# teofum/yart

Measured on AMD Instinct MI355X. Metric: Msamples/sec (W*H*spp/s), Sponza-class 1080p 8-bounce, higher is better.
Workload: dtype f32; 1 GPU; sponza_class (generated atrium, 264356 triangles, env-lit) 1920x1080, 256 spp, 8 bounces; pipeline=wavefront, tiles=64x64 pixel blocks, Morton order, round-robin over ranks, pipeline_flags=2

## Files before the change

### yart_amd/csrc/stream_kernels.inc

```

struct SamplerTabArgs {
  SamplerConfig cfg;
  const uint32_t* pixels; uint32_t nPixels, dims;
  uint64_t* entries; uint64_t* hash; uint32_t* sobol1;
  const uint32_t* matrix52;
};
__global__ void __launch_bounds__(kBlock) k_sampler_tables(SamplerTabArgs a) {
  const uint32_t gtid = blockIdx.x * blockDim.x + threadIdx.x, stride = gridDim.x * blockDim.x;
  for (uint32_t k = gtid; k < a.dims + 3u; k += stride) a.hash[k] = hashDim(k);
  for (uint32_t k = gtid; k < 8u * 256u; k += stride) {
    const uint32_t b = k >> 8, v = k & 255u;
    uint32_t x = 0;
    for (uint32_t j = 0; j < 8; j++) if (((v >> j) & 1u) && 8u * b + j < 52u) x ^= a.matrix52[8u * b + j];
    a.sobol1[k] = x;
  }
  const uint64_t total = uint64_t(a.dims) * a.nPixels;
  for (uint64_t k = gtid; k < total; k += stride) {
    const uint32_t pi = uint32_t(k / a.dims), dim = uint32_t(k - uint64_t(pi) * a.dims);
    const uint32_t pk = a.pixels[pi];
    a.entries[k] = samplerTableEntry(a.cfg, encodeMorton2(pk & 0xffffu, pk >> 16), dim);
  }
}

__global__ void __launch_bounds__(kBlock) k_wf_generate(WfArgs a) {
  WF_DYN(a);
  const uint32_t* sobol = reinterpret_cast<const uint32_t*>(a.sc.lut + LutDev::sobol);
  __shared__ SamplerLds smpLds;
  samplerToLds(a.rc.sampler, smpLds, true);
  for (uint32_t i = blockIdx.x * blockDim.x + threadIdx.x; i < a.nPaths; i += gridDim.x * blockDim.x) {
    const uint32_t pi = i / a.spp, s = i - pi * a.spp;
    const uint32_t pk = a.pixels[pi];
    wfGenerate(a.rc, sobol, a.cam, pk & 0xffffu, pk >> 16, s + a.sampleOffset, a.pixBase + pi, a.st, i);
    a.qA[i] = i;
  }
}

__global__ void __launch_bounds__(kBlock) k_wf_refill(WfArgs a) {
  const uint32_t* sobol = reinterpret_cast<const uint32_t*>(a.sc.lut + LutDev::sobol);
  __shared__ SamplerLds smpLds;
  samplerToLds(a.rc.sampler, smpLds, true);
  const uint32_t lane = threadIdx.x & 63u;
  const uint32_t waveId = (blockIdx.x * blockDim.x + threadIdx.x) >> 6, nWaves = (gridDim.x * blockDim.x) >> 6;
  const uint32_t per = (((a.poolSlots + nWaves - 1u) / nWaves) + 63u) & ~63u;
  const uint32_t s0 = waveId * per < a.poolSlots ? waveId * per : a.poolSlots, s1 = s0 + per < a.poolSlots ? s0 + per : a.poolSlots;
  uint32_t nFree = 0;
  for (uint32_t base = s0; base < s1; base += 64u) {
    const uint32_t slot = base + lane;
    nFree += uint32_t(__popcll(__ballot(slot < s1 && a.slotMap[slot] == kWfFreeSlot)));
  }
  uint32_t first = 0, avail = 0;
  if (nFree != 0u && a.counters[WC_STARTED] < a.nPaths) {
    if (lane == 0) first = atomicAdd(&a.counters[WC_STARTED], nFree);
    first = __shfl(first, 0);
    avail = first < a.nPaths ? (a.nPaths - first < nFree ? a.nPaths - first : nFree) : 0u;
  }
  uint32_t taken = 0;
  for (uint32_t base = s0; base < s1; base += 64u) {
    const uint32_t slot = base + lane;
    const bool isFree = slot < s1 && a.slotMap[slot] == kWfFreeSlot;
    const unsigned long long m = __ballot(isFree);
    const uint32_t k = taken + uint32_t(__popcll(m & ((1ull << lane) - 1ull)));
    const bool take = isFree && k < avail;
    if (take) {
      const uint32_t i = first + k;
      const uint32_t pi = i / a.spp, sm = i - pi * a.spp;
      const uint32_t pk = a.pixels[pi];
      wfGenerate(a.rc, sobol, a.cam, pk & 0xffffu, pk >> 16, sm + a.sampleOffset, a.pixBase + pi, a.st, slot);
      a.slotMap[slot] = i;
    }
    if (slot < s1) a.qA[slot] = (isFree && !take) ? kWfFreeSlot : slot;
    taken += uint32_t(__popcll(m));
  }
  const uint32_t live = (s1 - s0) - nFree + avail;
  if (lane == 0 && live != 0u) atomicAdd(&a.counters[WC_NEXT], live);
}
__global__ void k_wf_pool_advance(uint32_t* counters, uint32_t poolSlots) {
  if (threadIdx.x == 0 && blockIdx.x == 0) {
    counters[WC_ACTIVE] = poolSlots;
    for (uint32_t k = 1; k < WC_COUNT; k++) if (k != WC_STARTED) counters[k] = 0;
  }
}
__global__ void k_wf_pool_init(uint32_t* slotMap, uint32_t n) {
  for (uint32_t i = blockIdx.x * blockDim.x + threadIdx.x; i < n; i += gridDim.x * blockDim.x) slotMap[i] = kWfFreeSlot;
}

__global__ void k_wf_reset_retry(uint32_t* counters) {
  if (threadIdx.x == 0 && blockIdx.x == 0) { counters[WC_RETRY] = 0; counters[WC_CUR_RETRY] = 0; counters[WC_RESUME] = 0; }
}

#ifndef YART_COMPACT_NUM
#define YART_COMPACT_NUM 1
#define YART_COMPACT_DEN 2
#endif
__device__ __forceinline__ bool wfCompactPlan(const WfArgs& a, const WfDyn& d, uint32_t count, uint32_t& dst) {
  dst = d.inTail == 1u ? 1u : 0u;
  return count > 0u && count <= a.tailCap[dst] && uint64_t(YART_COMPACT_DEN) * count <= uint64_t(YART_COMPACT_NUM) * d.extent;
}
__global__ void __launch_bounds__(kBlock) k_wf_compact(WfArgs a) {
  const WfDyn d = *a.dyn;
  const uint32_t count = a.counters[WC_ACTIVE];
  uint32_t dst;
  if (!wfCompactPlan(a, d, count, dst)) return;
  const WfState from = d.st, to = a.tail[dst];
  uint32_t* map = a.tailMap[dst];
  const uint32_t stride = gridDim.x * blockDim.x;
  for (uint32_t k0 = blockIdx.x * blockDim.x + threadIdx.x; k0 < count; k0 += 2u * stride) {
    const uint32_t k1 = k0 + stride;
    const bool v1 = k1 < count;
    const uint32_t s0 = a.qA[k0], s1 = v1 ? a.qA[k1] : s0;
    const f4 a0 = wfLd(from.ray0 + s0), b0 = wfLd(from.ray1 + s0), c0 = wfLd(from.thr + s0), d0 = wfLd(from.acc + s0), e0 = wfLd(from.hit1 + s0);
    const f4 a1 = wfLd(from.ray0 + s1), b1 = wfLd(from.ray1 + s1), c1 = wfLd(from.thr + s1), d1 = wfLd(from.acc + s1), e1 = wfLd(from.hit1 + s1);
    const uint32_t m0 = d.slotMap ? d.slotMap[s0] : s0, m1 = d.slotMap ? d.slotMap[s1] : s1;
    wfSt(to.ray0 + k0, a0); wfSt(to.ray1 + k0, b0); wfSt(to.thr + k0, c0); wfSt(to.acc + k0, d0); wfSt(to.hit1 + k0, e0);
    map[k0] = m0; a.qA[k0] = k0;
    if (v1) {
      wfSt(to.ray0 + k1, a1); wfSt(to.ray1 + k1, b1); wfSt(to.thr + k1, c1); wfSt(to.acc + k1, d1); wfSt(to.hit1 + k1, e1);
      map[k1] = m1; a.qA[k1] = k1;
    }
  }
}
__global__ void k_wf_compact_commit(WfArgs a) {
  if (threadIdx.x != 0 || blockIdx.x != 0) return;
  const WfDyn d = *a.dyn;
  const uint32_t count = a.counters[WC_ACTIVE];
  uint32_t dst;
  if (!wfCompactPlan(a, d, count, dst)) return;
  WfDyn n;
  n.st = a.tail[dst]; n.slotMap = a.tailMap[dst]; n.extent = count; n.inTail = dst + 1u;
  *a.dyn = n;
}

__global__ void k_wf_advance(uint32_t* counters, unsigned long long* pathsLog) {
  if (threadIdx.x == 0 && blockIdx.x == 0) {
    counters[0] = counters[1];
    if (pathsLog) *pathsLog += counters[1] - counters[WC_DUMMY];
    for (uint32_t k = 1; k < WC_COUNT; k++) if (k != WC_STARTED) counters[k] = 0;
  }
}

__global__ void __launch_bounds__(kBlock) k_wf_roulette(WfArgs a) {
  WF_EMPTY_BLOCK(a.counters[WC_SHADOW], kBlock);
  WF_DYN(a);
  const uint32_t count = a.counters[WC_SHADOW];
  const uint32_t stride = gridDim.x * blockDim.x;
  const uint32_t rounds = (count + stride - 1) / stride;
  __shared__ uint32_t stageNext[kBlock / 64][kStageCap];
  WaveStage sNext{stageNext[threadIdx.x >> 6], 0};
  __shared__ SamplerLds smpLds;
  samplerToLds(a.rc.sampler, smpLds, false);
  for (uint32_t r = 0; r < rounds; r++) {
    const uint32_t k = r * stride + blockIdx.x * blockDim.x + threadIdx.x;
    bool toNext = false;
    uint32_t slot = 0;
    if (k < count) {
      slot = a.qS[k];
      if (a.poolSlots) {
        const uint32_t fl = asU(wfLd1(&a.st.acc[slot].w));
        if ((fl & WF_DEPTH_MASK) >= 2u && !(fl & WF_FINAL)) toNext = wfRouletteAfterShadow(a.rc, a.st, slot, fl & WF_DEPTH_MASK, a.L, a.slotMap, true);
      } else toNext = wfRouletteAfterShadow(a.rc, a.st, slot, a.bounce + 1u, a.L, a.slotMap, false);
    }
    if (!a.poolSlots) sNext.push(a.qB, &a.counters[WC_NEXT], toNext, slot);
  }
  sNext.flush(a.qB, &a.counters[WC_NEXT]);
}
```

### yart_amd/csrc/wavefront.hpp

```cpp
#pragma once
#include "integrator.hpp"

namespace yart_hip {

struct WfState {
  f4 *ray0, *ray1, *thr, *acc, *hit0, *hit1, *sh0, *sh1, *sh2;
};
struct WfTally {
#if defined(YART_COUNT_TRAVERSAL)
  uint32_t box = 0, tri = 0, trav = 0, shade = 0;
  uint32_t resumed = 0;
  uint32_t waste = 0;
  uint32_t flipAlive = 0, flipDead = 0;
#endif
#if defined(YART_TRACE_STATS)
  uint32_t ph[16] = {0, 0, 0, 0, 0, 0, 0, 0, 0, 0, 0, 0, 0, 0, 0, 0};
#endif
};
#if defined(YART_TRACE_STATS)
#define WF_PHASE(t, k)                                                                  \
  do {                                                                                  \
    const unsigned long long _m = __ballot(true);                                       \
    (t).ph[2 * (k)] += (int(threadIdx.x & 63u) == __ffsll((long long) _m) - 1) ? 1u : 0u; \
    (t).ph[2 * (k) + 1] += 1u;                                                          \
  } while (0)
#else
#define WF_PHASE(t, k) ((void)0)
#endif
#if defined(YART_COUNT_TRAVERSAL)
#define WF_TALLY_TRAV(t, ac) ((t).box += (ac).nBox, (t).tri += (ac).nTri, (t).trav += (ac).nTrav)
#define WF_TALLY_SHADE(t) ((t).shade++)
#define WF_TALLY_FLIP(t, toAlive) ((toAlive) ? (t).flipAlive++ : (t).flipDead++)
#else
#define WF_TALLY_TRAV(t, ac) ((void)0)
#define WF_TALLY_SHADE(t) ((void)0)
#define WF_TALLY_FLIP(t, toAlive) ((void)0)
#endif

#if defined(YART_SHADE_REGIONS) && defined(__HIPCC__)
constexpr int kShadeRegions = 16;
static __device__ unsigned long long g_shadeRegion[3 * kShadeRegions];
#endif
#if defined(YART_SHADE_REGIONS) && defined(__HIP_DEVICE_COMPILE__)
__shared__ unsigned long long srAcc[16][3 * kShadeRegions];
__shared__ unsigned long long srLast[16];
#define SR_MARK(k)                                                                       \
  do {                                                                                   \
    const unsigned long long _m = __ballot(true);                                        \
    if (int(threadIdx.x & 63u) == __ffsll((long long) _m) - 1) {                         \
      const unsigned long long _t = clock64();                                           \
      unsigned long long* _a = srAcc[threadIdx.x >> 6];                                  \
      _a[k] += _t - srLast[threadIdx.x >> 6]; _a[kShadeRegions + (k)] += 1ull;           \
      _a[2 * kShadeRegions + (k)] += (unsigned long long) __popcll(_m);                  \
      srLast[threadIdx.x >> 6] = clock64();                                              \
    }                                                                                    \
  } while (0)
#else
#define SR_MARK(k) ((void)0)
#endif

enum : uint32_t { WF_SPECULAR = 1u << 8, WF_REGULARIZED = 1u << 9, WF_MISS = 1u << 10, WF_DEPTH_MASK = 0xffu,
                  WF_NEE_SHIFT = 16, WF_NEE_ONE = 1u << 16, WF_NEE_MASK = 0xffu << 16,
                  WF_FINAL = 1u << 11, WF_ATT_NAN = 1u << 12,
                  WF_RR_PENDING = 1u << 13, WF_DEAD = 1u << 14 };

constexpr uint32_t kWfNodeBits = 20, kWfClassBits = 11, kWfClassMiss = (1u << kWfClassBits) - 1u;
YART_HD uint32_t wfHitWord(const HitRec& h, bool didHit) {
  if (!didHit) return kWfClassMiss << kWfNodeBits;
  return h.node | ((h.backSide >> 1) << kWfNodeBits) | ((h.backSide & 1u) << 31);
}
YART_HD float asF(uint32_t u) { return __builtin_bit_cast(float, u); }
YART_HD uint32_t asU(float f) { return __builtin_bit_cast(uint32_t, f); }
YART_HD f4 mk4(float x, float y, float z, float w) { f4 r; r.x = x; r.y = y; r.z = z; r.w = w; return r; }

#if defined(__HIP_DEVICE_COMPILE__) && !defined(YART_NO_NT_STATE)
typedef float wf_v4 __attribute__((ext_vector_type(4)));
typedef __attribute__((address_space(1))) wf_v4 wf_v4_global;
typedef __attribute__((address_space(1))) float wf_f_global;
__device__ __forceinline__ f4 wfLd(const f4* p) {
  const wf_v4 v = __builtin_nontemporal_load((const wf_v4_global*) reinterpret_cast<const wf_v4*>(p));
  return mk4(v.x, v.y, v.z, v.w);
}
__device__ __forceinline__ void wfSt(f4* p, f4 v) {
  wf_v4 q; q.x = v.x; q.y = v.y; q.z = v.z; q.w = v.w;
  __builtin_nontemporal_store(q, (wf_v4_global*) reinterpret_cast<wf_v4*>(p));
}
__device__ __forceinline__ void wfSt1(float* p, float v) { __builtin_nontemporal_store(v, (wf_f_global*) p); }
__device__ __forceinline__ float wfLd1(const float* p) { return *(const wf_f_global*) p; }
#else
YART_HD f4 wfLd(const f4* p) { return *p; }
YART_HD void wfSt(f4* p, f4 v) { *p = v; }
YART_HD void wfSt1(float* p, float v) { *p = v; }
YART_HD float wfLd1(const float* p) { return *p; }
#endif

struct WfPath {
  f3 o, d, att, L;
  float lastPdf, accRoughness;
  uint32_t flags, slot;
  Sampler smp;
};
YART_HD WfPath wfLoad(const WfState& s, uint32_t i) {
  const f4 r0 = wfLd(s.ray0 + i), r1 = wfLd(s.ray1 + i), t = wfLd(s.thr + i), a = wfLd(s.acc + i), h1 = wfLd(s.hit1 + i);
  WfPath p;
  p.o = mk3(r0.x, r0.y, r0.z); p.d = mk3(r0.w, r1.x, r1.y); p.lastPdf = r1.z; p.accRoughness = r1.w;
  p.att = mk3(t.x, t.y, t.z); p.smp.dim = asU(t.w); p.L = mk3(a.x, a.y, a.z); p.flags = asU(a.w);
  p.smp.morton = uint64_t(asU(h1.y)) | (uint64_t(asU(h1.z)) << 32); p.smp.pix = asU(h1.w); p.slot = i;
  return p;
}
YART_HD void wfStoreRay(const WfState& s, uint32_t i, const WfPath& p) {
  wfSt(s.ray0 + i, mk4(p.o.x, p.o.y, p.o.z, p.d.x));
  wfSt(s.ray1 + i, mk4(p.d.y, p.d.z, p.lastPdf, p.accRoughness));
}
YART_HD void wfStoreThr(const WfState& s, uint32_t i, const WfPath& p) {
  wfSt(s.thr + i, mk4(p.att.x, p.att.y, p.att.z, asF(p.smp.dim)));
  wfSt(s.acc + i, mk4(p.L.x, p.L.y, p.L.z, asF(p.flags)));
}
YART_HD uint32_t wfPathRays(uint32_t flags) { return (flags & WF_DEPTH_MASK) + ((flags & WF_NEE_MASK) >> WF_NEE_SHIFT); }

YART_HD bool wfRoulette(const RenderConst& rc, WfPath& p) {
  const uint32_t depth = p.flags & WF_DEPTH_MASK;
  if (depth > 1 && maxComponent(p.att) < 1.0f) {
    float q = stdmax(0.0f, 1.0f - maxComponent(p.att));
    if (get1D(p.smp, rc.sampler) < q) return false;
    p.att /= 1.0f - q;
  }
  return depth < rc.maxDepth;
}
YART_HD bool wfRouletteTentative(const RenderConst& rc, WfPath& p) {
  if (!(maxComponent(p.att) < 1.0f)) return true;
  const float q = stdmax(0.0f, 1.0f - maxComponent(p.att));
  p.flags |= WF_RR_PENDING;
  if (get1D(p.smp, rc.sampler) < q) { p.flags |= WF_FINAL; return false; }
  return true;
}
YART_HD void wfRouletteScale(f3& att) {
  const float q = stdmax(0.0f, 1.0f - maxComponent(att));
  att /= 1.0f - q;
}

YART_HD void wfGenerate(const RenderConst& rc, const uint32_t* sobol, const CameraDev& cam, uint32_t px,
                        uint32_t py, uint32_t sample, uint32_t pix, const WfState& s, uint32_t i) {
  WfPath p;
  startPixelSample(p.smp, rc.sampler, px, py, sample);
  p.smp.pix = pix;
  f2 uvFilm = get2D(p.smp, rc.sampler, sobol);
  f2 uvLens = get2D(p.smp, rc.sampler, sobol);
  cameraRay(cam, px, py, uvFilm, uvLens, p.o, p.d);
  p.att = mk3(1.0f); p.L = mk3(0.0f); p.lastPdf = 0.0f; p.accRoughness = 0.0f; p.flags = 0; p.slot = i;
  wfStoreRay(s, i, p);
  wfStoreThr(s, i, p);
  s.hit1[i] = mk4(0.0f, asF(uint32_t(p.smp.morton)), asF(uint32_t(p.smp.morton >> 32)), asF(pix));
}

constexpr uint32_t kWfFreeSlot = 0xffffffffu;
YART_HD void wfRetire(f4* out, uint32_t* slotMap, uint32_t slot, f4 record, bool pool) {
  uint32_t idx = slot;
  if (slotMap) { idx = slotMap[slot]; if (pool) slotMap[slot] = kWfFreeSlot; }
  wfSt(out + idx, record);
}
YART_HD bool wfRouletteAfterShadow(const RenderConst& rc, const WfState& s, uint32_t slot, uint32_t depth, f4* out, uint32_t* slotMap, bool pool) {
  const f4 t = wfLd(s.thr + slot);
  WfPath p;
  p.att = mk3(t.x, t.y, t.z);
  if (!(maxComponent(p.att) < 1.0f)) return true;
  const f4 h1 = wfLd(s.hit1 + slot);
  p.smp.dim = asU(t.w); p.smp.morton = uint64_t(asU(h1.y)) | (uint64_t(asU(h1.z)) << 32); p.smp.pix = asU(h1.w);
  p.flags = depth;
  if (wfRoulette(rc, p)) {
    wfSt(s.thr + slot, mk4(p.att.x, p.att.y, p.att.z, asF(p.smp.dim)));
    return true;
  }
  const f4 a = wfLd(s.acc + slot);
  wfRetire(out, slotMap, slot, mk4(a.x, a.y, a.z, asF(wfPathRays(asU(a.w)))), pool);
  return false;
}


YART_HD uint32_t wfShadowCommitLoaded(const WfState& s, uint32_t slot, f4 a, uint32_t flags, bool flagsChanged, bool occluded, f3 attOcc,
                                      f4* out, uint32_t* slotMap, bool pool, const f4* sh12 = nullptr) {
  if (occluded && !(flags & (WF_FINAL | WF_ATT_NAN))) {
    if (flagsChanged) wfSt1(&s.acc[slot].w, asF(flags));
    return 0u;
  }
  f3 L = mk3(a.x, a.y, a.z);
  if (!occluded) {
    const f4 s1 = sh12 ? sh12[0] : wfLd(s.sh1 + slot), s2 = sh12 ? sh12[1] : wfLd(s.sh2 + slot);
    L += mk3(s1.x, s1.y, s1.z) * (mk3(s2.x, s2.y, s2.z) * attOcc * s2.w / s1.w);
    flags += WF_NEE_ONE;
  } else if (flags & WF_ATT_NAN) {
    const f4 s1 = wfLd(s.sh1 + slot);
    L += mk3(s1.x, s1.y, s1.z) * mk3(0.0f);
  }
  if (flags & WF_FINAL) wfRetire(out, slotMap, slot, mk4(L.x, L.y, L.z, asF(wfPathRays(flags))), pool);
  else wfSt(s.acc + slot, mk4(L.x, L.y, L.z, asF(flags)));
  return occluded ? 0u : 1u;
}
YART_HD uint32_t wfShadowCommit(const WfState& s, uint32_t slot, bool occluded, f3 attOcc, f4* out, uint32_t* slotMap, bool pool) {
  const f4 a = wfLd(s.acc + slot);
  return wfShadowCommitLoaded(s, slot, a, asU(a.w), false, occluded, attOcc, out, slotMap, pool);
}
template <class Repair>
YART_HD uint32_t wfShadowCommitGeneral(const SamplerConfig& cfg, const WfState& s, uint32_t slot, bool occluded, f3 attOcc, uint32_t dim0,
                                       uint32_t dim, f4* out, uint32_t* slotMap, bool pool, Repair& repair, WfTally& tally) {
  const f4 a = wfLd(s.acc + slot), t = wfLd(s.thr + slot), h1 = wfLd(s.hit1 + slot);
  f4 sh12[2] = {a, a};
  if (!occluded) { sh12[0] = wfLd(s.sh1 + slot); sh12[1] = wfLd(s.sh2 + slot); }
  uint32_t flags = asU(a.w);
  bool flagsChanged = false;
  if (dim != dim0 && !(flags & WF_RR_PENDING)) wfSt1(&s.thr[slot].w, asF(dim));
  else if (dim != dim0) {
    Sampler smp;
    smp.dim = dim; smp.morton = uint64_t(asU(h1.y)) | (uint64_t(asU(h1.z)) << 32); smp.pix = asU(h1.w);
    const float q = stdmax(0.0f, 1.0f - maxComponent(mk3(t.x, t.y, t.z)));
    const bool dies = get1D(smp, cfg) < q, wasDead = (flags & WF_FINAL) != 0u;
    if (!dies) wfSt1(&s.thr[slot].w, asF(smp.dim));
    if (wasDead && !dies) {
      flags &= ~uint32_t(WF_FINAL); flagsChanged = true;
      if (!pool) repair.revived(slot);
      WF_TALLY_FLIP(tally, true);
    } else if (!wasDead && dies) {
      flags |= WF_FINAL;
      wfSt1(&s.acc[slot].w, asF(flags | WF_DEAD));
      if (!pool) repair.died();
      WF_TALLY_FLIP(tally, false);
    }
  }
  return wfShadowCommitLoaded(s, slot, a, flags, flagsChanged, occluded, attOcc, out, slotMap, pool, occluded ? nullptr : sh12);
}

YART_HD void wfExtend(const SceneDev& sc, const RenderConst& rc, const TravStack& stk, const WfState& s,
                      uint32_t i, WfTally& tally) {
  const f4 r0 = s.ray0[i], r1 = s.ray1[i];
  f4 h1 = s.hit1[i];
  Sampler smp;
  smp.dim = asU(s.thr[i].w);
  smp.morton = uint64_t(asU(h1.y)) | (uint64_t(asU(h1.z)) << 32); smp.pix = asU(h1.w);
  const uint32_t dim0 = smp.dim;
  HitRec hr;
  hr.t = kInf; hr.u = hr.v = 0; hr.tri = 0; hr.node = 0; hr.backSide = 0;
  f3 dummy = mk3(1.0f);
  AlphaCtx ac; ac.sampler = &smp; ac.cfg = rc.sampler;
  bool hit = traverseScene<false>(sc, mk3(r0.x, r0.y, r0.z), mk3(r0.w, r1.x, r1.y), 0.001f, hr, dummy, stk, ac);
  WF_TALLY_TRAV(tally, ac);
  s.hit0[i] = mk4(hit ? hr.t : -1.0f, hr.u, hr.v, asF(hr.tri));
  h1.x = asF(wfHitWord(hr, hit));
  s.hit1[i] = h1;
  if (smp.dim != dim0) s.thr[i].w = asF(smp.dim);
}

template <int MODE>
YART_HD bool wfExtendFast(const SceneDev& sc, const TravStack& stk, const WfState& s, uint32_t i, WfTally& tally) {
  const f4 r0 = s.ray0[i], r1 = s.ray1[i];
  HitRec hr;
  hr.t = kInf; hr.u = hr.v = 0; hr.tri = 0; hr.node = 0; hr.backSide = 0;
  f3 dummy = mk3(1.0f);
  AlphaCtx ac; ac.sampler = nullptr; ac.cfg = SamplerConfig{};
  const bool hit = traverseScene<false, MODE>(sc, mk3(r0.x, r0.y, r0.z), mk3(r0.w, r1.x, r1.y), 0.001f, hr, dummy, stk, ac);
  WF_TALLY_TRAV(tally, ac);
  if (ac.deferred) return false;
  s.hit0[i] = mk4(hit ? hr.t : -1.0f, hr.u, hr.v, asF(hr.tri));
  s.hit1[i].x = asF(wfHitWord(hr, hit));
  return true;
}

struct WfNoRepair { YART_HD void revived(uint32_t) {} YART_HD void died() {} };
template <int MODE, class Repair>
YART_HD bool wfShadow(const SceneDev& sc, const RenderConst& rc, const TravStack& stk, const WfState& s,
                      uint32_t i, WfTally& tally, f4* out, uint32_t* slotMap, bool pool, uint32_t& rays, Repair& repair) {
  const f4 r0 = s.ray0[i], s0 = s.sh0[i];
  const f3 from = mk3(r0.x, r0.y, r0.z), to = mk3(s0.x, s0.y, s0.z);
  const f3 dir = normalized(to - from);
  HitRec hr;
  hr.t = length(to - from) - 0.001f;
  hr.u = hr.v = 0; hr.tri = 0; hr.node = 0; hr.backSide = 0;
  f3 attOcc = mk3(1.0f);
  Sampler smp; smp.dim = 0; smp.morton = 0;
  AlphaCtx ac; ac.sampler = &smp; ac.cfg = rc.sampler;
  if (!(MODE & TRAV_FAST)) {
    const f4 h1 = s.hit1[i];
    smp.dim = asU(s0.w);
    smp.morton = uint64_t(asU(h1.y)) | (uint64_t(asU(h1.z)) << 32); smp.pix = asU(h1.w);
  }
  const bool occluded = traverseScene<true, MODE>(sc, from, dir, 0.001f, hr, attOcc, stk, ac);
  WF_TALLY_TRAV(tally, ac);
  if ((MODE & TRAV_FAST) && ac.deferred) return false;
  if (MODE & TRAV_FAST) rays += wfShadowCommit(s, i, occluded, attOcc, out, slotMap, pool);
  else rays += wfShadowCommitGeneral(rc.sampler, s, i, occluded, attOcc, asU(s0.w), smp.dim, out, slotMap, pool, repair, tally);
  return true;
}

enum WfShadeResult { WF_TERMINATED = 0, WF_CONTINUE = 1, WF_SHADOW = 2, WF_SKIPPED = 3 };

YART_HD WfShadeResult wfShade(const SceneDev& sc, const RenderConst& rc, const uint32_t* sobol, const WfState& s,
                              uint32_t i, WfPath& p, uint32_t& rays, WfTally& tally) {
  p = wfLoad(s, i);
  if (p.flags & WF_DEAD) return WF_SKIPPED;
  if (p.flags & WF_RR_PENDING) wfRouletteScale(p.att);
  const f4 h0 = wfLd(s.hit0 + i);
  const uint32_t nodeBack = asU(s.hit1[i].x);
  const uint32_t depth = p.flags & WF_DEPTH_MASK;
  const bool specularBounce = (p.flags & WF_SPECULAR) != 0, regularized = (p.flags & WF_REGULARIZED) != 0;
  rays++;
  SR_MARK(0);
  if (h0.x < 0.0f) {
    for (uint32_t k = 0; k < sc.nInfinite; k++) {
      const LightDev& l = sc.lights[sc.infiniteLights[k]];
      f3 Le = lightLe(sc, l, octahedralUV(p.d));
      if (depth == 0 || specularBounce) p.L += p.att * Le;
      else {
        float pdfLight = lightPdf(sc, l, p.d);
        float wBSDF = p.lastPdf / (p.lastPdf + pdfLight);
        p.L += p.att * wBSDF * Le;
      }
    }
    p.L += p.att * rc.background;
    SR_MARK(1);
    return WF_TERMINATED;
  }
  HitRec hr;
  hr.t = h0.x; hr.u = h0.y; hr.v = h0.z; hr.tri = asU(h0.w); hr.node = nodeBack & ((1u << kWfNodeBits) - 1u);
  hr.backSide = (nodeBack >> 31) | (((nodeBack >> kWfNodeBits) & kWfClassMiss) << 1);
  Hit hit = finalizeHit(sc, hr, p.o, p.d);
  SR_MARK(2);
  WF_TALLY_SHADE(tally);
  const MaterialDev& mt = sc.materials[hit.material];
  f2 u = get2D(p.smp, rc.sampler, sobol);
  float uc = get1D(p.smp, rc.sampler);
  Sampler smpUc2 = p.smp;
  p.smp.dim++;
  SR_MARK(3);
  const f3 wo = -p.d;
  const Frame fr = shadingFrame(hit.n, hit.tg);
  const f3 woLocal = wtl(fr, wo);
  const MatEval me = matEvaluate(sc, mt, hit.uv);
  float uc2 = 0.0f;
  if (!(me.c == 0.0f && me.m == 0.0f && me.t == 0.0f)) uc2 = get1D(smpUc2, rc.sampler);
  SR_MARK(4);
  BsdfSample res = bsdfSampleImplE(sc, mt, me, woLocal, hit.uv, u, uc, uc2, regularized);
  res.wi = ltw(fr, res.wi);
  SR_MARK(5);
  if (res.scatter & SC_EMITTED) {
    if (depth == 0 || specularBounce) p.L += p.att * res.Le;
    else if (hit.lightIdx != -1) {
      const LightDev& l = sc.lights[hit.lightIdx];
      float pdfLight = lightPdf(sc, l, wo) * length2(p.o - hit.p) * lightSamplerP(sc, uint32_t(hit.lightIdx)) /
                       absDot(wo, hit.n);
      float wBSDF = p.lastPdf / (p.lastPdf + pdfLight);
      p.L += p.att * wBSDF * res.Le;
    }
  }
  if (!(res.scatter & (SC_REFLECTED | SC_TRANSMITTED))) return WF_TERMINATED;

  const f3 fcos = res.f * absDot(res.wi, hit.n);
  f3 newAtt = p.att * (fcos / res.pdf);
  if (hit.backSide) newAtt *= matAttenuation(mt, hit.t);
  {
    WfPath q;
    q.o = hit.p; q.d = res.wi; q.lastPdf = res.pdf; q.accRoughness = p.accRoughness + res.roughness;
    wfStoreRay(s, i, q);
    uint32_t fl = ((depth + 1) & WF_DEPTH_MASK) | (p.flags & WF_NEE_MASK);
    if (res.scatter & SC_SPECULAR) fl |= WF_SPECULAR;
    if (q.accRoughness > 0.5f) fl |= WF_REGULARIZED;
    p.flags = fl;
  }
  SR_MARK(6);
  const bool nee = !(res.scatter & (SC_EMITTED | SC_SPECULAR));

  bool shadow = false;
  if (nee) {
    if (sc.nLights != 0) {
      float ucl = 0.0f;
      if (sc.nArea == 0u && sc.nInfinite == 1u) p.smp.dim++;
      else ucl = get1D(p.smp, rc.sampler);
      f2 ul = get2D(p.smp, rc.sampler, sobol);
      SR_MARK(7);
      float pl;
      uint32_t li = lightSamplerSample(sc, ucl, pl);
      const LightDev& l = sc.lights[li];
      LightSample ls = lightSample(sc, l, hit.p, ul);
      const f3 wiLocal = wtl(fr, ls.wi);
      SR_MARK(8);
      f3 f = bsdfFImplE(sc, mt, me, woLocal, wiLocal);
      SR_MARK(9);
      if (length2(f) != 0.0f) {
        float pdfBSDF = bsdfPdfImplE(sc, mt, me, woLocal, wiLocal);
        float pdfLight = pl * ls.pdf / absDot(ls.n, ls.wi);
        if (l.type == LIGHT_AREA) pdfLight *= length2(hit.p - ls.p);
        const f3 Lif = ls.Li * f;
        wfSt(s.sh0 + i, mk4(ls.p.x, ls.p.y, ls.p.z, asF(p.smp.dim)));
        wfSt(s.sh1 + i, mk4(p.att.x, p.att.y, p.att.z, pdfBSDF + pdfLight));
        wfSt(s.sh2 + i, mk4(Lif.x, Lif.y, Lif.z, absDot(ls.wi, hit.n)));
        shadow = true;
        if ((p.flags & WF_DEPTH_MASK) >= rc.maxDepth) p.flags |= WF_FINAL;
        {
          const f3 z = p.att * mk3(0.0f);
          if (!(z.x == 0.0f && z.y == 0.0f && z.z == 0.0f)) p.flags |= WF_ATT_NAN;
        }
        SR_MARK(10);
      }
    }
    if (!shadow) p.L += p.att * mk3(0.0f);
  }
  p.att = newAtt;
  return shadow ? WF_SHADOW : WF_CONTINUE;
}

}
```

### yart_amd/csrc/wavefront_kernels.inc

```

constexpr int kWfLdsStack = 16;
#ifndef YART_LEAN_LDS_STACK
#define YART_LEAN_LDS_STACK 8
#endif
#ifndef YART_LEAN_WAVES
#define YART_LEAN_WAVES 7
#endif
constexpr int leanWaves(int) { return YART_LEAN_WAVES; }
constexpr int kWfLdsStackFast = YART_LEAN_LDS_STACK;
constexpr int kWfSpillDepth = int(kRefStackDepth) - kWfLdsStack;
#ifndef YART_WF_MAX_PATHS_LOG2
#define YART_WF_MAX_PATHS_LOG2 30
#endif
constexpr uint32_t kWfMaxPaths = 1u << YART_WF_MAX_PATHS_LOG2;

struct WfDyn {
  WfState st;
  uint32_t* slotMap;
  uint32_t extent;
  uint32_t inTail;
};
struct WfArgs {
  SceneDev sc;
  CameraDev cam;
  RenderConst rc;
  WfDyn* dyn;
  uint32_t* slotMap;
  WfState tail[2];
  uint32_t* tailMap[2];
  uint32_t tailCap[2];
  WfState st;
  uint32_t* qA;
  uint32_t* qB;
  uint32_t* qS;
  uint32_t* qR;
  uint32_t* counters;
  const uint32_t* pixels;
  uint32_t nPaths, spp, sampleOffset, pixBase;
  uint32_t bounce;
  f4* L;
  unsigned long long* stats;
  uint64_t* spill;
  f4* resumeRec;
  uint32_t resumeCap, padR;
  const uint8_t* matClass;
  uint32_t poolSlots, padP;
};

enum WfCounter : uint32_t {
  WC_ACTIVE = 0, WC_NEXT = 1, WC_SHADOW = 2, WC_CUR_EXTEND = 3, WC_CUR_SHADE = 4, WC_CUR_SHADOW = 5,
  WC_RETRY = 6, WC_CUR_RETRY = 7,
  WC_RESUME = 8,
  WC_STARTED = 9,
  WC_DUMMY = 10,
  WC_COUNT = 11
};

#define WF_EMPTY_BLOCK(count, per) do { if (uint64_t(blockIdx.x) * uint64_t(per) >= uint64_t(count)) return; } while (0)
#define WF_DYN(a) do { if ((a).dyn) { (a).st = (a).dyn->st; (a).slotMap = (a).dyn->slotMap; } } while (0)

__device__ __forceinline__ void wfPush(uint32_t* q, uint32_t* counter, bool pred, uint32_t slot) {
  const unsigned long long m = __ballot(pred);
  if (m == 0) return;
  const uint32_t lane = threadIdx.x & 63u;
  const int leader = __ffsll((long long) m) - 1;
  uint32_t base = 0;
  if (int(lane) == leader) base = atomicAdd(counter, uint32_t(__popcll(m)));
  base = __shfl(base, leader);
  if (pred) q[base + __popcll(m & ((1ull << lane) - 1ull))] = slot;
}

constexpr uint32_t kStageCap = 512;
template <uint32_t CAP>
struct WaveStageT {
  uint32_t* buf;
  uint32_t n;
  __device__ __forceinline__ void flush(uint32_t* q, uint32_t* counter) {
    if (n == 0) return;
    const uint32_t lane = threadIdx.x & 63u;
    uint32_t base = 0;
    if (lane == 0) base = atomicAdd(counter, n);
    base = __shfl(base, 0);
    for (uint32_t i = lane; i < n; i += 64u) q[base + i] = buf[i];
    n = 0;
  }
  __device__ __forceinline__ void push(uint32_t* q, uint32_t* counter, bool pred, uint32_t slot) {
    const unsigned long long m = __ballot(pred);
    if (m == 0) return;
    const uint32_t lane = threadIdx.x & 63u;
    if (pred) buf[n + __popcll(m & ((1ull << lane) - 1ull))] = slot;
    n += uint32_t(__popcll(m));
    if (n > CAP - 64u) flush(q, counter);
  }
};
typedef WaveStageT<kStageCap> WaveStage;
__device__ __forceinline__ void ldsCopyWords(uint32_t* dst, const void* src, uint32_t words) {
  const uint32_t* s = reinterpret_cast<const uint32_t*>(src);
  for (uint32_t k = threadIdx.x; k < words; k += blockDim.x) dst[k] = s[k];
}
struct SamplerLds { uint64_t hash[264]; uint32_t sobol1[8 * 256]; };
__device__ __forceinline__ void samplerToLds(SamplerConfig& c, SamplerLds& l, bool sobol) {
  if (c.tab.hash == nullptr || c.tab.dims + 3u > 264u) return;
  for (uint32_t k = threadIdx.x; k < c.tab.dims + 3u; k += blockDim.x) l.hash[k] = c.tab.hash[k];
  if (sobol) for (uint32_t k = threadIdx.x; k < 8u * 256u; k += blockDim.x) l.sobol1[k] = c.tab.sobol1[k];
  __syncthreads();
  c.tab.hash = l.hash;
  if (sobol) c.tab.sobol1 = l.sobol1;
}
constexpr uint32_t kLeanSceneNodes = 16;
struct LeanSceneLds { uint32_t node[kLeanSceneNodes * sizeof(NodeDev) / 4], world[kLeanSceneNodes * 8], mesh[kLeanSceneNodes * sizeof(MeshDev) / 4]; };
__device__ __forceinline__ void leanSceneToLds(SceneDev& sc, LeanSceneLds& l, uint32_t nMeshes) {
  ldsCopyWords(l.node, sc.nodes, sc.nNodes * uint32_t(sizeof(NodeDev) / 4));
  ldsCopyWords(l.world, sc.nodeWorld, sc.nNodes * 8u);
  ldsCopyWords(l.mesh, sc.meshes, nMeshes * uint32_t(sizeof(MeshDev) / 4));
  __syncthreads();
  sc.nodes = reinterpret_cast<const NodeDev*>(l.node); sc.nodeWorld = reinterpret_cast<const f4*>(l.world);
  sc.meshes = reinterpret_cast<const MeshDev*>(l.mesh);
}
constexpr uint32_t kRepairCap = 32;
struct WfRepairLds { uint32_t slots[kBlock / 64][kRepairCap]; uint32_t n[kBlock / 64]; };
struct WfRepair {
  uint32_t* slots; uint32_t* n;
  uint32_t* qNext; uint32_t* counters;
  uint32_t dummies;
  __device__ __forceinline__ WfRepair(WfRepairLds& l, uint32_t* q, uint32_t* c) : slots(l.slots[threadIdx.x >> 6]), n(&l.n[threadIdx.x >> 6]), qNext(q), counters(c), dummies(0) {
    if ((threadIdx.x & 63u) == 0) *n = 0;
  }
  __device__ __forceinline__ void revived(uint32_t slot) {
    const uint32_t i = atomicAdd(n, 1u);
    if (i < kRepairCap) slots[i] = slot;
    else qNext[atomicAdd(&counters[WC_NEXT], 1u)] = slot;
  }
  __device__ __forceinline__ void died() { dummies++; }
  __device__ __forceinline__ void flush() {
    const uint32_t lane = threadIdx.x & 63u;
    const uint32_t count = *n < kRepairCap ? *n : kRepairCap;
    if (count != 0u) {
      uint32_t base = 0;
      if (lane == 0) base = atomicAdd(&counters[WC_NEXT], count);
      base = __shfl(base, 0);
      for (uint32_t i = lane; i < count; i += 64u) qNext[base + i] = slots[i];
    }
    uint32_t d = dummies;
    for (int o = 32; o > 0; o >>= 1) d += __shfl_down(d, o);
    if (lane == 0 && d) atomicAdd(&counters[WC_DUMMY], d);
  }
};
constexpr uint32_t kRetryStageCap = 128;

__device__ __forceinline__ void wfWriteL(f4* L, uint32_t slot, f3 v, uint32_t rays) { wfSt(L + slot, mk4(v.x, v.y, v.z, asF(rays))); }

__device__ __forceinline__ void wfAddStat(unsigned long long* p, uint32_t v) {
  unsigned long long r = v;
  for (int o = 32; o > 0; o >>= 1) r += __shfl_down(r, o);
  if ((threadIdx.x & 63u) == 0 && r) atomicAdd(p, r);
}

__device__ __forceinline__ void wfFlushTally(unsigned long long* stats, const WfTally& t) {
#if defined(YART_COUNT_TRAVERSAL)
  wfAddStat(stats + 1, t.trav); wfAddStat(stats + 2, t.box); wfAddStat(stats + 3, t.tri); wfAddStat(stats + 4, t.shade);
#else
  (void)stats; (void)t;
#endif
#if defined(YART_TRACE_STATS)
  for (int k = 0; k < 16; k++) wfAddStat(stats + 8 + k, t.ph[k]);
#endif
}

template <int LDS_DEPTH, bool RETRY_INPUT, bool LEAN_EXTEND, class Trace>
__device__ __forceinline__ void wfTraverseQueue(const WfArgs& a, const uint32_t* q, uint32_t count, uint32_t* cursor,
                                                uint64_t* ldsStack, Trace trace) {
  const uint32_t lane = threadIdx.x & 63u;
  const uint32_t gtid = blockIdx.x * blockDim.x + threadIdx.x;
  TravStack stk;
  stk.lds = (lds_u64*)(ldsStack + threadIdx.x); stk.ldsStride = kBlock; stk.ldsDepth = LDS_DEPTH;
  stk.spill = a.spill + gtid; stk.spillStride = gridDim.x * blockDim.x;
  __shared__ uint32_t stageRetry[kBlock / 64][RETRY_INPUT ? 1 : kRetryStageCap];
  WaveStageT<kRetryStageCap> sRetry{stageRetry[threadIdx.x >> 6], 0};
  WfTally tally;
  const uint32_t nWaves = (gridDim.x * blockDim.x) >> 6;
  const uint32_t chunk = leanChunk(count, nWaves);
  uint32_t next = 0, end = 0;
  for (uint32_t base = (gtid >> 6) * 64u; base < count;) {
    const uint32_t k = base + lane;
    bool retry = false;
    uint32_t slot = 0;
    if (k < count) { slot = q[k]; if (slot != kWfFreeSlot) retry = trace(stk, slot, tally); }
    if (!RETRY_INPUT) sRetry.push(a.qR, &a.counters[WC_RETRY], retry, slot);
    if (next == end) {
      uint32_t c = 0;
      if (lane == 0) c = atomicAdd(cursor, chunk);
      next = nWaves * 64u + __shfl(c, 0);
      end = next + chunk;
    }
    base = next;
    next += 64u;
  }
  if (!RETRY_INPUT) sRetry.flush(a.qR, &a.counters[WC_RETRY]);
  wfFlushTally(a.stats, tally);
#if defined(YART_COUNT_TRAVERSAL)
  if (LEAN_EXTEND) { wfAddStat(a.stats + 5, tally.trav); wfAddStat(a.stats + 6, tally.box); wfAddStat(a.stats + 7, tally.tri); }
  wfAddStat(a.stats + 10, tally.flipAlive); wfAddStat(a.stats + 11, tally.flipDead);
#endif
}

template <int MODE>
__global__ void __launch_bounds__(kBlock, 6) k_wf_extend_fast(WfArgs a) {
  WF_DYN(a);
  __shared__ uint64_t ldsStack[kWfLdsStackFast * kBlock];
  wfTraverseQueue<kWfLdsStackFast, false, true>(a, a.qA, a.counters[WC_ACTIVE], &a.counters[WC_CUR_EXTEND], ldsStack,
      [&](const TravStack& stk, uint32_t slot, WfTally& tally) { return !wfExtendFast<MODE>(a.sc, stk, a.st, slot, tally); });
}
template <bool RETRY>
__global__ void __launch_bounds__(kBlock, 4) k_wf_extend(WfArgs a) {
  WF_DYN(a);
  __shared__ uint64_t ldsStack[kWfLdsStack * kBlock];
  wfTraverseQueue<kWfLdsStack, true, false>(a, RETRY ? a.qR : a.qA, a.counters[RETRY ? WC_RETRY : WC_ACTIVE],
      &a.counters[RETRY ? WC_CUR_RETRY : WC_CUR_EXTEND], ldsStack,
      [&](const TravStack& stk, uint32_t slot, WfTally& tally) { wfExtend(a.sc, a.rc, stk, a.st, slot, tally); return false; });
}
template <int MODE>
__global__ void __launch_bounds__(kBlock, 6) k_wf_shadow_fast(WfArgs a) {
  WF_DYN(a);
  __shared__ uint64_t ldsStack[kWfLdsStackFast * kBlock];
  uint32_t rays = 0;
  wfTraverseQueue<kWfLdsStackFast, false, false>(a, a.qS, a.counters[WC_SHADOW], &a.counters[WC_CUR_SHADOW], ldsStack,
      [&](const TravStack& stk, uint32_t slot, WfTally& tally) { WfNoRepair none; return !wfShadow<MODE>(a.sc, a.rc, stk, a.st, slot, tally, a.L, a.slotMap, a.poolSlots != 0u, rays, none); });
  wfAddStat(a.stats, rays);
}
template <bool RETRY>
__global__ void __launch_bounds__(kBlock, 4) k_wf_shadow(WfArgs a) {
  WF_DYN(a);
  __shared__ uint64_t ldsStack[kWfLdsStack * kBlock];
  uint32_t rays = 0;
  __shared__ WfRepairLds repairLds;
  WfRepair repair(repairLds, a.qB, a.counters);
  wfTraverseQueue<kWfLdsStack, true, false>(a, RETRY ? a.qR : a.qS, a.counters[RETRY ? WC_RETRY : WC_SHADOW],
      &a.counters[RETRY ? WC_CUR_RETRY : WC_CUR_SHADOW], ldsStack,
      [&](const TravStack& stk, uint32_t slot, WfTally& tally) {
        wfShadow<TRAV_GENERAL>(a.sc, a.rc, stk, a.st, slot, tally, a.L, a.slotMap, a.poolSlots != 0u, rays, repair);
        return false;
      });
  repair.flush();
  wfAddStat(a.stats, rays);
}
template <int MODE, int NODES>
__global__ void __launch_bounds__(kBlock, leanWaves(MODE)) k_wf_extend_lean(WfArgs a) {
  WF_EMPTY_BLOCK(a.counters[WC_ACTIVE], kBlock);
  WF_DYN(a);
  __shared__ uint64_t ldsStack[kWfLdsStackFast * kBlock];
  __shared__ uint32_t stageRetry[kBlock / 64][kRetryStageCap];
  const uint32_t gtid = blockIdx.x * blockDim.x + threadIdx.x;
  TravStack stk;
  stk.lds = (lds_u64*)(ldsStack + threadIdx.x); stk.ldsStride = kBlock; stk.ldsDepth = kWfLdsStackFast;
  stk.spill = a.spill + gtid; stk.spillStride = gridDim.x * blockDim.x;
  WaveStageT<kRetryStageCap> sRetry{stageRetry[threadIdx.x >> 6], 0};
  WfTally tally;
  const WfState st = a.st;
  stk.rec = a.resumeRec; stk.recCursor = &a.counters[WC_RESUME]; stk.recCap = a.resumeCap;
  __shared__ __attribute__((aligned(16))) LeanSceneLds sceneLds;
  if (NODES == kNodesMaskLds) leanSceneToLds(a.sc, sceneLds, a.sc.nMeshes);
  traceLeanAny<false, MODE, NODES>(a.sc, a.rc.sampler, stk, a.qA, a.counters[WC_ACTIVE], &a.counters[WC_CUR_EXTEND],
      [&](uint32_t slot) {
        const f4 r0 = wfLd(st.ray0 + slot), r1 = wfLd(st.ray1 + slot);
        LeanRay r; r.o = mk3(r0.x, r0.y, r0.z); r.d = mk3(r0.w, r1.x, r1.y); r.tMax = kInf;
        return r;
      },
      [&](uint32_t slot, const HitRec& h, bool didHit, f3, uint32_t) {
        wfSt(st.hit0 + slot, mk4(didHit ? h.t : -1.0f, h.u, h.v, asF(h.tri)));
        wfSt1(&st.hit1[slot].x, asF(wfHitWord(h, didHit)));
      },
      [&](bool pred, uint32_t slot) { sRetry.push(a.qR, &a.counters[WC_RETRY], pred, slot); }, tally);
  sRetry.flush(a.qR, &a.counters[WC_RETRY]);
  wfFlushTally(a.stats, tally);
#if defined(YART_COUNT_TRAVERSAL)
  wfAddStat(a.stats + 5, tally.trav); wfAddStat(a.stats + 6, tally.box); wfAddStat(a.stats + 7, tally.tri);
  wfAddStat(a.stats + 27, tally.waste);
#endif
}
template <int MODE, int NODES>
__global__ void __launch_bounds__(kBlock, leanWaves(MODE)) k_wf_shadow_lean(WfArgs a) {
  WF_EMPTY_BLOCK(a.counters[WC_SHADOW], kBlock);
  WF_DYN(a);
  __shared__ uint64_t ldsStack[kWfLdsStackFast * kBlock];
  __shared__ uint32_t stageRetry[kBlock / 64][kRetryStageCap];
  const uint32_t gtid = blockIdx.x * blockDim.x + threadIdx.x;
  TravStack stk;
  stk.lds = (lds_u64*)(ldsStack + threadIdx.x); stk.ldsStride = kBlock; stk.ldsDepth = kWfLdsStackFast;
  stk.spill = a.spill + gtid; stk.spillStride = gridDim.x * blockDim.x;
  WaveStageT<kRetryStageCap> sRetry{stageRetry[threadIdx.x >> 6], 0};
  WfTally tally;
  const WfState st = a.st;
  uint32_t nRays = 0;
  stk.rec = a.resumeRec; stk.recCursor = &a.counters[WC_RESUME]; stk.recCap = a.resumeCap;
  __shared__ __attribute__((aligned(16))) LeanSceneLds sceneLds;
  if (NODES == kNodesMaskLds) leanSceneToLds(a.sc, sceneLds, a.sc.nMeshes);
  traceLeanAny<true, MODE, NODES>(a.sc, a.rc.sampler, stk, a.qS, a.counters[WC_SHADOW], &a.counters[WC_CUR_SHADOW],
      [&](uint32_t slot) {
        const f4 r0 = wfLd(st.ray0 + slot), s0 = wfLd(st.sh0 + slot);
        const f3 from = mk3(r0.x, r0.y, r0.z), to = mk3(s0.x, s0.y, s0.z);
        LeanRay r; r.o = from; r.d = normalized(to - from);
        r.tMax = length(to - from) - 0.001f;
        return r;
      },
      [&](uint32_t slot, const HitRec&, bool occluded, f3, uint32_t) {
        nRays += wfShadowCommit(st, slot, occluded, mk3(1.0f), a.L, a.slotMap, a.poolSlots != 0u);
      },
      [&](bool pred, uint32_t slot) { sRetry.push(a.qR, &a.counters[WC_RETRY], pred, slot); }, tally);
  sRetry.flush(a.qR, &a.counters[WC_RETRY]);
  wfAddStat(a.stats, nRays);
  wfFlushTally(a.stats, tally);
#if defined(YART_COUNT_TRAVERSAL)
  wfAddStat(a.stats + 24, tally.trav); wfAddStat(a.stats + 25, tally.box); wfAddStat(a.stats + 26, tally.tri);
  wfAddStat(a.stats + 31, tally.waste);
#endif
}

#ifndef YART_RETRY_WAVES
#define YART_RETRY_WAVES 4
#endif
template <int NODES>
__global__ void __launch_bounds__(kBlock, YART_RETRY_WAVES) k_wf_extend_retry_lean(WfArgs a) {
  WF_EMPTY_BLOCK(a.counters[WC_RETRY], kBlock);
  WF_DYN(a);
  __shared__ uint64_t ldsStack[kWfLdsStack * kBlock];
  const uint32_t gtid = blockIdx.x * blockDim.x + threadIdx.x;
  TravStack stk;
  stk.lds = (lds_u64*)(ldsStack + threadIdx.x); stk.ldsStride = kBlock; stk.ldsDepth = kWfLdsStack;
  stk.spill = a.spill + gtid; stk.spillStride = gridDim.x * blockDim.x;
  WfTally tally;
  const WfState st = a.st;
  stk.rec = a.resumeRec; stk.recCursor = &a.counters[WC_RESUME]; stk.recCap = a.resumeCap;
  __shared__ __attribute__((aligned(16))) LeanSceneLds sceneLds;
  if (NODES == kNodesMaskLds) leanSceneToLds(a.sc, sceneLds, a.sc.nMeshes);
  __shared__ uint64_t sHash[264];
  if (a.rc.sampler.tab.hash != nullptr && a.rc.sampler.tab.dims + 3u <= 264u) {
    for (uint32_t k = threadIdx.x; k < a.rc.sampler.tab.dims + 3u; k += blockDim.x) sHash[k] = a.rc.sampler.tab.hash[k];
    __syncthreads();
    a.rc.sampler.tab.hash = sHash;
  }
  traceLeanAny<false, TRAV_GENERAL, NODES>(a.sc, a.rc.sampler, stk, a.qR, a.counters[WC_RETRY], &a.counters[WC_CUR_RETRY],
      [&](uint32_t slot) {
        const f4 r0 = wfLd(st.ray0 + slot), r1 = wfLd(st.ray1 + slot), h1 = wfLd(st.hit1 + slot);
        LeanRay r; r.o = mk3(r0.x, r0.y, r0.z); r.d = mk3(r0.w, r1.x, r1.y); r.tMax = kInf;
        r.smp.dim = asU(wfLd1(&st.thr[slot].w)); r.smp.morton = uint64_t(asU(h1.y)) | (uint64_t(asU(h1.z)) << 32); r.smp.pix = asU(h1.w);
        return r;
      },
      [&](uint32_t slot, const HitRec& h, bool didHit, f3, uint32_t dim) {
        wfSt(st.hit0 + slot, mk4(didHit ? h.t : -1.0f, h.u, h.v, asF(h.tri)));
        wfSt1(&st.hit1[slot].x, asF(wfHitWord(h, didHit)));
        wfSt1(&st.thr[slot].w, asF(dim));
      },
      [&](bool, uint32_t) {}, tally);
  wfFlushTally(a.stats, tally);
#if defined(YART_COUNT_TRAVERSAL)
  wfAddStat(a.stats + 29, tally.trav);
  wfAddStat(a.stats + 8, tally.resumed);
#endif
}
template <int NODES>
__global__ void __launch_bounds__(kBlock, YART_RETRY_WAVES) k_wf_shadow_retry_lean(WfArgs a) {
  WF_EMPTY_BLOCK(a.counters[WC_RETRY], kBlock);
  WF_DYN(a);
  __shared__ uint64_t ldsStack[kWfLdsStack * kBlock];
  const uint32_t gtid = blockIdx.x * blockDim.x + threadIdx.x;
  TravStack stk;
  stk.lds = (lds_u64*)(ldsStack + threadIdx.x); stk.ldsStride = kBlock; stk.ldsDepth = kWfLdsStack;
  stk.spill = a.spill + gtid; stk.spillStride = gridDim.x * blockDim.x;
  WfTally tally;
  const WfState st = a.st;
  uint32_t nRays = 0;
  stk.rec = a.resumeRec; stk.recCursor = &a.counters[WC_RESUME]; stk.recCap = a.resumeCap;
  __shared__ __attribute__((aligned(16))) LeanSceneLds sceneLds;
  if (NODES == kNodesMaskLds) leanSceneToLds(a.sc, sceneLds, a.sc.nMeshes);
  __shared__ uint64_t sHash[264];
  if (a.rc.sampler.tab.hash != nullptr && a.rc.sampler.tab.dims + 3u <= 264u) {
    for (uint32_t k = threadIdx.x; k < a.rc.sampler.tab.dims + 3u; k += blockDim.x) sHash[k] = a.rc.sampler.tab.hash[k];
    __syncthreads();
    a.rc.sampler.tab.hash = sHash;
  }
  __shared__ WfRepairLds repairLds;
  WfRepair repair(repairLds, a.qB, a.counters);
  traceLeanAny<true, TRAV_GENERAL, NODES>(a.sc, a.rc.sampler, stk, a.qR, a.counters[WC_RETRY], &a.counters[WC_CUR_RETRY],
      [&](uint32_t slot) {
        const f4 r0 = wfLd(st.ray0 + slot), s0 = wfLd(st.sh0 + slot), h1 = wfLd(st.hit1 + slot);
        const f3 from = mk3(r0.x, r0.y, r0.z), to = mk3(s0.x, s0.y, s0.z);
        LeanRay r; r.o = from; r.d = normalized(to - from); r.tMax = length(to - from) - 0.001f;
        r.smp.dim = asU(s0.w); r.smp.morton = uint64_t(asU(h1.y)) | (uint64_t(asU(h1.z)) << 32); r.smp.pix = asU(h1.w);
        return r;
      },
      [&](uint32_t slot, const HitRec&, bool occluded, f3 att, uint32_t dim) {
        nRays += wfShadowCommitGeneral(a.rc.sampler, st, slot, occluded, att, asU(wfLd1(&st.sh0[slot].w)), dim, a.L, a.slotMap, a.poolSlots != 0u,
                                       repair, tally);
      },
      [&](bool, uint32_t) {}, tally);
  repair.flush();
  wfAddStat(a.stats, nRays);
  wfFlushTally(a.stats, tally);
#if defined(YART_COUNT_TRAVERSAL)
  wfAddStat(a.stats + 30, tally.trav);
  wfAddStat(a.stats + 9, tally.resumed);
  wfAddStat(a.stats + 10, tally.flipAlive); wfAddStat(a.stats + 11, tally.flipDead);
#endif
}

#ifndef YART_SHADE_WAVES
#define YART_SHADE_WAVES 3
#endif
constexpr int kShadeBlock = YART_SHADE_WAVES * 256;
constexpr uint32_t kShadeStageCap = 512;
constexpr int kShadeBlocksPerCU = 1;
constexpr uint32_t kShadeHashSlots = 264, kShadeMatSlots = 64, kShadeTexSlots = 128, kShadeLightSlots = 8, kShadeEnvSlots = 4, kShadeNodeSlots = 32;
template <bool SORT, bool FIT, bool ENV1>
__global__ void __launch_bounds__(kShadeBlock, kShadeBlocksPerCU) k_wf_shade(WfArgs a) {
  WF_EMPTY_BLOCK(a.counters[0], kShadeBlock * 4);
  WF_DYN(a);
  if (ENV1) { __builtin_assume(a.sc.nArea == 0u); __builtin_assume(a.sc.nInfinite == 1u); __builtin_assume(a.sc.nLights == 1u); }
  const uint32_t lane = threadIdx.x & 63u;
  const unsigned long long laneLt = (1ull << lane) - 1ull;
  const uint32_t* sobol = reinterpret_cast<const uint32_t*>(a.sc.lut + LutDev::sobol);
  const uint32_t count = a.counters[0];
  uint32_t rays = 0;
  WfTally tally;
  __shared__ uint32_t stageNext[kShadeBlock / 64][kShadeStageCap], stageShadow[kShadeBlock / 64][kShadeStageCap];
  __shared__ uint32_t sorted[kShadeBlock / 64][SORT ? 256 : 1];
  WaveStageT<kShadeStageCap> sNext{stageNext[threadIdx.x >> 6], 0}, sShadow{stageShadow[threadIdx.x >> 6], 0};
  uint32_t* mySorted = sorted[threadIdx.x >> 6];
  const uint32_t waveId = (blockIdx.x * blockDim.x + threadIdx.x) >> 6, nWaves = (gridDim.x * blockDim.x) >> 6;
  uint32_t nSorted = 0;
  __shared__ uint64_t sHash[kShadeHashSlots];
  __shared__ uint32_t sSobol1[8 * 256];
  if (FIT || (a.rc.sampler.tab.hash != nullptr && a.rc.sampler.tab.dims + 3u <= kShadeHashSlots)) {
    for (uint32_t k = threadIdx.x; k < a.rc.sampler.tab.dims + 3u; k += blockDim.x) sHash[k] = a.rc.sampler.tab.hash[k];
    for (uint32_t k = threadIdx.x; k < 8u * 256u; k += blockDim.x) sSobol1[k] = a.rc.sampler.tab.sobol1[k];
    __syncthreads();
    a.rc.sampler.tab.hash = sHash; a.rc.sampler.tab.sobol1 = sSobol1;
  }
  __shared__ float sLut[LutDev::glassE + 2];
  {
    const float* g = a.sc.lut;
    for (uint32_t k = threadIdx.x; k < LutDev::glassE; k += blockDim.x) sLut[k] = g[k];
    if (threadIdx.x == 0) {
      const uint64_t p = reinterpret_cast<uint64_t>(g);
      reinterpret_cast<uint32_t*>(sLut)[LutDev::glassE] = uint32_t(p); reinterpret_cast<uint32_t*>(sLut)[LutDev::glassE + 1] = uint32_t(p >> 32);
    }
    __syncthreads();
    a.sc.lut = sLut;
  }
  {
    constexpr uint32_t kMatCap = kShadeMatSlots, kTexCap = kShadeTexSlots, kLightCap = kShadeLightSlots, kEnvCap = kShadeEnvSlots, kNodeCap = kShadeNodeSlots, kInfCap = kShadeLightSlots;
    __shared__ __attribute__((aligned(16))) uint32_t sMat[kMatCap * sizeof(MaterialDev) / 4], sTex[kTexCap * sizeof(TexDev) / 4],
        sLight[kLightCap * sizeof(LightDev) / 4], sEnv[kEnvCap * sizeof(EnvDev) / 4], sNode[kNodeCap * sizeof(NodeDev) / 4], sInf[kInfCap],
        sClass[kMatCap / 4];
    const bool mOk = FIT || a.sc.nMaterials <= kMatCap, tOk = FIT || a.sc.nTextures <= kTexCap, lOk = FIT || (a.sc.nLights <= kLightCap && a.sc.nLights > 0u),
               eOk = FIT || a.sc.nEnvs <= kEnvCap, nOk = FIT || a.sc.nNodes <= kNodeCap, iOk = FIT || (a.sc.nInfinite <= kInfCap && a.sc.nInfinite > 0u);
    if (mOk) { ldsCopyWords(sMat, a.sc.materials, a.sc.nMaterials * uint32_t(sizeof(MaterialDev) / 4)); ldsCopyWords(sClass, a.matClass, (a.sc.nMaterials + 3u) / 4u); }
    if (tOk) ldsCopyWords(sTex, a.sc.textures, a.sc.nTextures * uint32_t(sizeof(TexDev) / 4));
    if (lOk) ldsCopyWords(sLight, a.sc.lights, a.sc.nLights * uint32_t(sizeof(LightDev) / 4));
    if (eOk) ldsCopyWords(sEnv, a.sc.envs, a.sc.nEnvs * uint32_t(sizeof(EnvDev) / 4));
    if (nOk) ldsCopyWords(sNode, a.sc.nodes, a.sc.nNodes * uint32_t(sizeof(NodeDev) / 4));
    if (iOk) ldsCopyWords(sInf, a.sc.infiniteLights, a.sc.nInfinite);
    __syncthreads();
    if (mOk) { a.sc.materials = reinterpret_cast<const MaterialDev*>(sMat); a.matClass = reinterpret_cast<const uint8_t*>(sClass); }
    if (tOk) a.sc.textures = reinterpret_cast<const TexDev*>(sTex);
    if (lOk) a.sc.lights = reinterpret_cast<const LightDev*>(sLight);
    if (eOk) a.sc.envs = reinterpret_cast<const EnvDev*>(sEnv);
    if (nOk) a.sc.nodes = reinterpret_cast<const NodeDev*>(sNode);
    if (iOk) a.sc.infiniteLights = sInf;
  }
#if defined(YART_SHADE_REGIONS) && defined(__HIP_DEVICE_COMPILE__)
  if (lane == 0) { for (int k = 0; k < 3 * kShadeRegions; k++) srAcc[threadIdx.x >> 6][k] = 0; srLast[threadIdx.x >> 6] = clock64(); }
#endif
  for (uint32_t sub = 0, grab = waveId * 256u, first = 1;; sub = (sub + 1u) & 3u) {
    if (sub == 0) {
      if (!first) {
        if (lane == 0) grab = atomicAdd(&a.counters[4], 256u);
        grab = nWaves * 256u + __shfl(grab, 0);
      }
      if (SORT && grab < count) {
        uint32_t slots[4], keys[4];
        unsigned long long pending[4];
        for (int r = 0; r < 4; r++) {
          const uint32_t k = grab + uint32_t(r) * 64u + lane;
          const uint32_t word = k < count ? a.qA[k] : kWfFreeSlot;
          const bool valid = word != kWfFreeSlot;
          slots[r] = valid ? word : 0u;
          if (valid) {
            const uint32_t m = (asU(wfLd1(&a.st.hit1[slots[r]].x)) >> kWfNodeBits) & kWfClassMiss;
            keys[r] = m == kWfClassMiss ? 0xffu : uint32_t(a.matClass[m]);
          } else keys[r] = 0xffffffffu;
          pending[r] = __ballot(valid);
        }
        uint32_t out = 0;
        while (pending[0] | pending[1] | pending[2] | pending[3]) {
          uint32_t key = 0;
          for (int r = 3; r >= 0; r--)
            if (pending[r]) key = __shfl(keys[r], __ffsll((long long) pending[r]) - 1);
          for (int r = 0; r < 4; r++) {
            const unsigned long long m = __ballot(keys[r] == key) & pending[r];
            if ((m >> lane) & 1ull) mySorted[out + uint32_t(__popcll(m & laneLt))] = slots[r];
            out += uint32_t(__popcll(m));
            pending[r] &= ~m;
          }
        }
        nSorted = out;
      }
    }
    first = 0;
    SR_MARK(12);
    const uint32_t base = grab + sub * 64u;
    if (base >= count) break;
    const uint32_t k = base + lane;
    bool toNext = false, toShadow = false;
    uint32_t slot = 0;
    const bool valid = SORT ? (sub * 64u + lane < nSorted) : (k < count && a.qA[k] != kWfFreeSlot);
    if (valid) {
      slot = SORT ? mySorted[sub * 64u + lane] : a.qA[k];
      WfPath p;
      WfShadeResult r = wfShade(a.sc, a.rc, sobol, a.st, slot, p, rays, tally);
      if (r == WF_SHADOW) {
        toShadow = true;
        if (p.flags & WF_FINAL) toNext = false;
        else if ((p.flags & WF_DEPTH_MASK) <= 1u) toNext = true;
        else toNext = !a.poolSlots && wfRouletteTentative(a.rc, p);
        wfStoreThr(a.st, slot, p);
      } else if (r == WF_CONTINUE && wfRoulette(a.rc, p)) {
        wfStoreThr(a.st, slot, p);
        toNext = true;
      } else if (r != WF_SKIPPED) {
        const uint32_t segs = (p.flags & WF_DEPTH_MASK) + (r == WF_TERMINATED ? 1u : 0u);
        wfRetire(a.L, a.slotMap, p.slot, mk4(p.L.x, p.L.y, p.L.z, asF(segs + ((p.flags & WF_NEE_MASK) >> WF_NEE_SHIFT))), a.poolSlots != 0u);
      }
    }
    if (!a.poolSlots) sNext.push(a.qB, &a.counters[1], toNext, slot);
    sShadow.push(a.qS, &a.counters[2], toShadow, slot);
    SR_MARK(11);
  }
  sNext.flush(a.qB, &a.counters[1]);
  sShadow.flush(a.qS, &a.counters[2]);
#if defined(YART_SHADE_REGIONS) && defined(__HIP_DEVICE_COMPILE__)
  if (lane == 0) for (int k = 0; k < 3 * kShadeRegions; k++) if (srAcc[threadIdx.x >> 6][k]) atomicAdd(&g_shadeRegion[k], srAcc[threadIdx.x >> 6][k]);
#endif
  wfAddStat(a.stats, rays);
  wfFlushTally(a.stats, tally);
#if defined(YART_COUNT_TRAVERSAL)
  wfAddStat(a.stats + 28, rays);
#endif
}
```

### yart_amd/csrc/yart_hip.hip

```cpp
#include "hip_common.hpp"

#include <algorithm>
#include <chrono>
#include <cstdio>
#include <functional>
#include <memory>
#include <mutex>
#include <string>
#include <type_traits>
#include <vector>

#include "../../include/yart_hip.h"
#include "estimator.hpp"
#include "host_scene.hpp"
#include "mesh_update.hpp"
#include "integrator.hpp"
#include "scene_file.hpp"
#include "gltf_reader.hpp"
#include "wavefront.hpp"
#include "trace_lean.hpp"
#include "moments.hpp"
#include "trace_ranges.hpp"
#include "kernel_units.hpp"

using namespace yart_hip;

namespace {

constexpr uint64_t kDefaultBatchPaths = 1ull << 28;
constexpr uint64_t kDefaultPoolPaths = 1ull << 25;
constexpr int kPoolLag = 4;

thread_local std::string g_lastError;

struct MegaArgs {
  SceneDev sc;
  CameraDev cam;
  RenderConst rc;
  const uint32_t* pixels;
  uint32_t nPixels, spp, sampleOffset, pad;
  f4* L;
  uint32_t* cursor;
  unsigned long long* rays;
  uint64_t* spill;
  f4 *aov0, *aov1, *aov2;
  int32_t* aovIds;
  uint32_t pixBase, padA;
};

template <bool AOV>
__global__ void __launch_bounds__(kBlock) k_render_mega(MegaArgs a) {
  __shared__ uint64_t ldsStack[kLdsStack * kBlock];
  const uint32_t lane = threadIdx.x & 63u;
  const uint32_t gtid = blockIdx.x * blockDim.x + threadIdx.x;
  const uint32_t nthreads = gridDim.x * blockDim.x;
  PathCtx cx;
  cx.sc = &a.sc;
  cx.sobol = reinterpret_cast<const uint32_t*>(a.sc.lut + LutDev::sobol);
  cx.stk.lds = (lds_u64*)(ldsStack + threadIdx.x); cx.stk.ldsStride = kBlock; cx.stk.ldsDepth = kLdsStack;
  cx.stk.spill = a.spill + gtid; cx.stk.spillStride = nthreads;
  cx.rc = a.rc;
  const uint32_t total = a.nPixels * a.spp;
  uint32_t rays = 0;
  for (;;) {
    uint32_t base = 0;
    if (lane == 0) base = atomicAdd(a.cursor, 64u);
    base = __shfl(base, 0);
    if (base >= total) break;
    const uint32_t w = base + lane;
    if (w < total) {
      const uint32_t pi = w / a.spp, s = w - pi * a.spp;
      const uint32_t pk = a.pixels[pi];
      const uint32_t before = rays;
      AovRecord rec; AovIds ids;
      f3 L = samplePixel<AOV>(cx, a.cam, pk & 0xffffu, pk >> 16, s + a.sampleOffset, rays, &rec, &ids);
      a.L[w] = mk4(L.x, L.y, L.z, asF(rays - before));
      if (AOV) {
        wfSt(a.aov0 + w, rec.r0); wfSt(a.aov1 + w, rec.r1); wfSt(a.aov2 + w, rec.r2);
        if (s + a.sampleOffset == 0u) {
          int32_t* o = a.aovIds + size_t(a.pixBase + pi) * 4;
          o[0] = ids.node; o[1] = ids.mesh; o[2] = ids.material; o[3] = ids.tri;
        }
      }
    }
  }
  unsigned long long r = rays;
  for (int o = 32; o > 0; o >>= 1) r += __shfl_down(r, o);
  if (lane == 0 && r) atomicAdd(a.rays, r);
#if defined(YART_COUNT_TRAVERSAL)
  unsigned long long c[4] = {cx.nTrav, cx.nBox, cx.nTri, cx.nShade};
  for (int k = 0; k < 4; k++) {
    unsigned long long v = c[k];
    for (int o = 32; o > 0; o >>= 1) v += __shfl_down(v, o);
    if (lane == 0 && v) atomicAdd(a.rays + 1 + k, v);
  }
#endif
}

struct GmonArgs {
  const f4* L;
  uint32_t* pixRays;
  const uint32_t* pixels;
  uint32_t nPixels, spp, width;
  int kind;
  float exposureScale, wCurrent, wWave, pad1;
  float* hdr;
};

constexpr int kGmonLanes = 16;
static_assert(kGmonMax <= kGmonLanes, "one lane per bucket");
constexpr int kGmonPixPerBlock = kBlock / kGmonLanes;
__global__ void __launch_bounds__(kBlock) k_gmon_blend(GmonArgs a) {
  __shared__ f3 sAcc[kGmonPixPerBlock][kGmonMax];
  __shared__ uint32_t sCnt[kGmonPixPerBlock][kGmonMax];
  const uint32_t sub = threadIdx.x & (kGmonLanes - 1), lp = threadIdx.x / kGmonLanes;
  const uint32_t pi = blockIdx.x * kGmonPixPerBlock + lp;
  const bool valid = pi < a.nPixels;
  const int m = estimatorBuckets(a.kind, int32_t(a.spp));
  __shared__ uint32_t sRays[kGmonPixPerBlock][kGmonMax];
  if (valid && int(sub) < m) {
    f3 acc = mk3(0); uint32_t cnt = 0, rays = 0;
    const f4* p = a.L + size_t(pi) * a.spp;
    const uint32_t um = uint32_t(m);
    uint32_t s = sub;
    for (; s + 3u * um < a.spp; s += 4u * um) {
      f4 v[4];
      for (uint32_t j = 0; j < 4u; j++) v[j] = p[s + j * um];
      for (uint32_t j = 0; j < 4u; j++) {
        const f3 w = mk3(v[j].x, v[j].y, v[j].z) * a.exposureScale;
        if (estimatorAccepts(a.kind, w)) { acc += w; cnt++; }
        rays += __builtin_bit_cast(uint32_t, v[j].w);
      }
    }
    for (; s < a.spp; s += um) {
      const f4 q = p[s];
      f3 v = mk3(q.x, q.y, q.z) * a.exposureScale;
      if (estimatorAccepts(a.kind, v)) { acc += v; cnt++; }
      rays += __builtin_bit_cast(uint32_t, q.w);
    }
    sAcc[lp][sub] = acc;
    sCnt[lp][sub] = cnt;
    sRays[lp][sub] = rays;
  }
  __syncthreads();
  if (valid && sub == 0 && a.pixRays != nullptr) {
    uint32_t r = 0;
    for (int b = 0; b < m; b++) r += sRays[lp][b];
    a.pixRays[pi] = r;
  }
  if (valid && sub == 0) {
    f3 v = estimatorFinish(a.kind, sAcc[lp], sCnt[lp], m, a.spp);
    const uint32_t pk = a.pixels[pi];
    float* o = a.hdr + (size_t(pk >> 16) * a.width + (pk & 0xffffu)) * 4;
    o[0] = o[0] * a.wCurrent + v.x * a.wWave;
    o[1] = o[1] * a.wCurrent + v.y * a.wWave;
    o[2] = o[2] * a.wCurrent + v.z * a.wWave;
    o[3] = o[3] * a.wCurrent + 1.0f * a.wWave;
  }
}

__global__ void __launch_bounds__(64) k_tile_rays(const uint32_t* pixRays, const uint32_t* tileStart, const uint32_t* tileCount,
                                                  uint32_t firstTile, uint32_t nTiles, unsigned long long* out) {
  const uint32_t t = firstTile + blockIdx.x;
  if (blockIdx.x >= nTiles) return;
  unsigned long long r = 0;
  for (uint32_t i = threadIdx.x; i < tileCount[t]; i += 64u) r += pixRays[tileStart[t] + i];
  for (int o = 32; o > 0; o >>= 1) r += __shfl_down(r, o);
  if (threadIdx.x == 0) out[t] = r;
}

struct TexQuadArgs { const uint8_t* u8; const float* f32; TexDev t; uint8_t* out; };
__global__ void __launch_bounds__(kBlock) k_tex_quads(TexQuadArgs a) {
  const uint32_t w = a.t.width, h = a.t.height, C = a.t.channels;
  const uint32_t rec = texQuadRecordBytes(C, a.t.isFloat);
  const uint32_t stride = a.t.quadStride ? a.t.quadStride : rec;
  const size_t n = size_t(w) * h;
  for (size_t i = size_t(blockIdx.x) * blockDim.x + threadIdx.x; i < n; i += size_t(gridDim.x) * blockDim.x) {
    const uint32_t x = uint32_t(i % w), y = uint32_t(i / w);
    const uint32_t x1 = x + 1u < w ? x + 1u : x, y1 = y + 1u < h ? y + 1u : y;
    const size_t idx[4] = {size_t(y) * w + x, size_t(y1) * w + x, size_t(y) * w + x1, size_t(y1) * w + x1};
    uint8_t* o = a.out + i * stride;
    if (a.t.isFloat) {
      float* of = reinterpret_cast<float*>(o);
      for (uint32_t k = 0; k < rec / 4u; k++) of[k] = 0.0f;
      for (uint32_t tap = 0; tap < 4u; tap++)
        for (uint32_t c = 0; c < C; c++) of[tap * C + c] = a.f32[size_t(a.t.offset) + C * idx[tap] + c];
    } else {
      uint32_t word[4];
      for (uint32_t tap = 0; tap < 4u; tap++) {
        word[tap] = 0u;
        for (uint32_t c = 0; c < C; c++) word[tap] |= uint32_t(a.u8[size_t(a.t.offset) + C * idx[tap] + c]) << (8u * c);
      }
      uint32_t* ow = reinterpret_cast<uint32_t*>(o);
      if (C >= 3u) { ow[0] = word[0]; ow[1] = word[1]; ow[2] = word[2]; ow[3] = word[3]; }
      else if (C == 2u) { ow[0] = word[0] | (word[1] << 16); ow[1] = word[2] | (word[3] << 16); }
      else ow[0] = word[0] | (word[1] << 8) | (word[2] << 16) | (word[3] << 24);
    }
  }
}

#include "wavefront_kernels.inc"
#include "stream_kernels.inc"
#include "aov_kernels.inc"
#include "moment_kernels.inc"
#include "bvh_build_device.inc"

static_assert(devbvh::kMaxLevels == int(kMaxStackBound), "the stack bound's cap is the device builder's level limit");
static size_t spillDepthFor(const HostImage& im, bool wholeStack) {
  if (wholeStack) return size_t(std::max<uint32_t>(uint32_t(kSpillDepthMax), im.stackBound));
  return size_t(std::max<int>(kSpillDepth, int(im.stackBound) - kLdsStack));
}
}
#include "render_host.hpp"
namespace {
typedef void (*WfKernelFn)(WfArgs);
inline WfKernelFn wfKernel(yart_hip::tu::AnyKernel k) { return reinterpret_cast<WfKernelFn>(k); }

struct Timer {
  hipEvent_t a{}, b{};
  Timer() { HIP_CHECK(hipEventCreate(&a)); HIP_CHECK(hipEventCreate(&b)); }
  ~Timer() { (void)hipEventDestroy(a); (void)hipEventDestroy(b); }
};

}

struct SceneUpdateTables {
  bool ready = false, tlasReady = false;
  uint32_t levels = 0;
  DevBuf<uint32_t> parents, childOff, childIdx;
  std::vector<uint32_t> levelFirst, levelBig, levelSmall;
  DevBuf<SuBox> meshBox;
  DevBuf<uint32_t> tlasOrder; std::vector<uint32_t> tlasFirst;
  DevBuf<uint32_t> stageDesc, stageFlags;
};

struct MeshStage {
  DevBuf<float> pos, nrm, tan;
  DevBuf<BvhNode> nodes; DevBuf<uint32_t> idx; DevBuf<LeafTri> leaf;
  std::vector<uint32_t> idxHost;
  uint32_t nNodes = 0, hasAlpha = 0, need = 0;
};
struct MeshUpdateState {
  devbvh::Scratch scratch;
  std::vector<std::unique_ptr<MeshStage>> stages;
  DevBuf<uint32_t> prefix, result;
  DevBuf<BvhNode> nodesAlt;
  std::vector<int8_t> meshAlpha;
};

struct YartScene {
  int device = 0;
  HostImage host;
  SceneDev dev{};
  int numCUs = 256;
  bool texQuadsOn = true;
  DevBuf<f4> resumeRec; DevBuf<ShadeTri> shadeTris; DevBuf<BvhNode> bvhNodes; DevBuf<LeafTri> leafTris; DevBuf<u4> triVerts; DevBuf<int32_t> triLight;
  DevBuf<f4> vPos, vNormal, vTangent; DevBuf<f2> vUV; DevBuf<MeshDev> meshes; DevBuf<NodeDev> nodes;
  DevBuf<MaterialDev> materials; DevBuf<TexDev> textures; DevBuf<uint8_t> texU8; DevBuf<float> texF32; DevBuf<uint8_t> texQuads;
  DevBuf<LightDev> lights; DevBuf<EnvDev> envs; DevBuf<float> envData; DevBuf<uint32_t> envGuide; DevBuf<f4> nodeWorld; DevBuf<TlasNode> tlas; DevBuf<unsigned long long> nodeBits;
  DevBuf<uint32_t> infiniteLights, areaLights; DevBuf<float> areaPowerCdf; DevBuf<float> lut;
  DevBuf<uint8_t> matClass;
  DevBuf<uint32_t> pixels; DevBuf<f4> L; DevBuf<uint32_t> cursor; DevBuf<unsigned long long> counters;
  DevBuf<uint32_t> pixRays, tileStart, tileCount; DevBuf<unsigned long long> tileRays;
  std::vector<unsigned long long> tileRaysHost;
  DevBuf<uint64_t> spill; DevBuf<float> hdr; DevBuf<uint32_t> probeIn; DevBuf<float> probeOut;
  DevBuf<f4> wf[9];
  DevBuf<f4> wfTail[1][9];
  DevBuf<uint32_t> wfTailMap[2];
  DevBuf<WfDyn> wfDyn;
  DevBuf<unsigned long long> pathsLog;
  DevBuf<f4> aovAcc[3], aovRec; DevBuf<uint32_t> aovRays; DevBuf<int32_t> aovIds; DevBuf<uint32_t> aovOut;
  DevBuf<MomentState> momState; DevBuf<uint32_t> momOut;
  DevBuf<uint32_t> poolMap;
  uint32_t* poolHost = nullptr;
  ~YartScene() { if (poolHost) (void)hipHostFree(poolHost); }
  DevBuf<uint32_t> qA, qB, qS, qR, wfCounters;
  DevBuf<uint64_t> smpEntries, smpHash; DevBuf<uint32_t> smpSobol1;
  std::vector<uint32_t> pixelsHost;
  struct TileRec { uint32_t x, y, w, h, start, count; };
  std::vector<TileRec> tiles;
  unsigned long long lastCounters[32] = {0};
  uint32_t pixW = 0, pixH = 0, pixTile = 0, pixRank = 0, pixWorld = 0;
  SceneUpdateTables su;
  MeshUpdateState meshUp;
  std::mutex mu;
};

namespace {

void uploadScene(YartScene& s) {
  const HostImage& h = s.host;
  s.shadeTris.upload(h.shadeTris);
  s.bvhNodes.upload(h.bvhNodes); s.leafTris.upload(h.leafTris); s.triVerts.upload(h.triVerts);
  s.triLight.upload(h.triLight); s.vPos.upload(h.vPos); s.vNormal.upload(h.vNormal);
  s.vTangent.upload(h.vTangent); s.vUV.upload(h.vUV); s.meshes.upload(h.meshes); s.nodes.upload(h.nodes);
  s.materials.upload(h.materials); s.textures.upload(h.textures); s.texU8.upload(h.texU8);
  s.texF32.upload(h.texF32); s.lights.upload(h.lights); s.envs.upload(h.envs); s.envData.upload(h.envData); s.envGuide.upload(h.envGuide); s.nodeWorld.upload(h.nodeWorld); s.tlas.upload(h.tlas);
  s.infiniteLights.upload(h.infiniteLights); s.areaLights.upload(h.areaLights);
  s.areaPowerCdf.upload(h.areaPowerCdf); s.lut.upload(h.lut);
  {
    std::vector<uint8_t> cls;
    for (const MaterialDev& m : h.materials) cls.push_back(lobeClass(m));
    while (cls.size() % 4u) cls.push_back(0);
    s.matClass.upload(cls);
  }
  bool quads = true;
  {
    size_t freeB = 0, totalB = 0;
    HIP_CHECK(hipMemGetInfo(&freeB, &totalB));
    size_t budget = freeB / 3;
    if (const char* e = std::getenv("YART_TEX_QUADS_MAX_MB")) budget = size_t(std::max<long long>(0, std::atoll(e))) << 20;
    if (h.texQuadUnits * 16u > budget) quads = false;
  }
  s.texQuadsOn = quads;
  s.texQuads.ensure(quads ? std::max<size_t>(h.texQuadUnits, 1) * 16u : 16u);
  for (const TexDev& t : h.textures) {
    if (!quads || t.width == 0u || t.quadOffset == kNoTexQuads) continue;
    TexQuadArgs qa{s.texU8.p, s.texF32.p, t, s.texQuads.p + size_t(t.quadOffset) * 16u};
    const size_t n = size_t(t.width) * t.height;
    hipLaunchKernelGGL(k_tex_quads, dim3(uint32_t(std::min<size_t>((n + kBlock - 1) / kBlock, 65535u))), dim3(kBlock), 0, nullptr, qa);
    HIP_CHECK(hipGetLastError());
  }
  HIP_CHECK(hipDeviceSynchronize());
  SceneDev d = h.view();
  d.shadeTris = s.shadeTris.p;
  d.bvhNodes = s.bvhNodes.p; d.leafTris = s.leafTris.p; d.triVerts = s.triVerts.p; d.triLight = s.triLight.p;
  d.vPos = s.vPos.p; d.vNormal = s.vNormal.p; d.vTangent = s.vTangent.p; d.vUV = s.vUV.p;
  d.meshes = s.meshes.p; d.nodes = s.nodes.p; d.materials = s.materials.p; d.textures = s.textures.p;
  d.texU8 = s.texU8.p; d.texF32 = s.texF32.p; d.texQuads = s.texQuadsOn ? s.texQuads.p : nullptr; d.lights = s.lights.p; d.envs = s.envs.p;
  d.envData = s.envData.p; d.envGuide = s.envGuide.p; d.nodeWorld = s.nodeWorld.p; d.tlas = s.tlas.p; d.nTlas = h.tlas.size() > 1 || (h.tlas.size() == 1 && h.tlas[0].b) ? uint32_t(h.tlas.size()) : 0u; d.infiniteLights = s.infiniteLights.p; d.areaLights = s.areaLights.p;
  d.areaPowerCdf = s.areaPowerCdf.p; d.lut = s.lut.p;
  s.dev = d;
}

int resolveDevice(int device) {
  int count = 0;
  hipError_t e = hipGetDeviceCount(&count);
  if (e != hipSuccess || count <= 0) return -1;
  if (device < 0) {
    int cur = 0;
    if (hipGetDevice(&cur) != hipSuccess) return -1;
    return cur;
  }
  return device < count ? device : -1;
}

static bool deviceMeshBvh(void* ctx, const float* positions, uint32_t nVerts, const uint32_t* faces, uint32_t stride, uint32_t nFaces,
                          std::vector<BvhNode>& nodes, std::vector<uint32_t>& indices) {
  try {
    return devbvh::build(*static_cast<int*>(ctx), positions, nVerts, faces, stride, nFaces, nodes, indices, nullptr);
  } catch (const std::exception&) {
    (void)hipGetLastError();
    nodes.clear(); indices.clear();
    return false;
  }
}
YartScene* createScene(const YartSceneDesc& desc, int device, uint32_t sceneFlags = 0) {
  int dev = resolveDevice(device);
  if (dev < 0) throw HipError("no usable HIP device (libyart_hip has no CPU fallback)");
  HIP_CHECK(hipSetDevice(dev));
  auto s = std::make_unique<YartScene>();
  s->device = dev;
  if ((sceneFlags & YART_SCENE_HOST_BVH) || std::getenv("YART_HOST_BVH")) s->host = buildHostImage(desc);
  else s->host = buildHostImage(desc, deviceMeshBvh, &dev);
  hipDeviceProp_t prop;
  HIP_CHECK(hipGetDeviceProperties(&prop, dev));
  s->numCUs = prop.multiProcessorCount;
  uploadScene(*s);
  return s.release();
}

uint32_t morton2(uint32_t x, uint32_t y) { return uint32_t(encodeMorton2(x, y)); }

std::vector<uint32_t> makePixelList(uint32_t W, uint32_t H, uint32_t tile, uint32_t rank, uint32_t world,
                                    std::vector<YartScene::TileRec>* tilesOut) {
  const uint32_t tx = (W + tile - 1) / tile, ty = (H + tile - 1) / tile;
  std::vector<std::pair<uint32_t, uint32_t>> order;
  for (uint32_t y = 0; y < ty; y++)
    for (uint32_t x = 0; x < tx; x++) order.push_back({morton2(x, y), y * tx + x});
  std::sort(order.begin(), order.end());
  std::vector<uint32_t> pixels;
  if (tilesOut) tilesOut->clear();
  for (size_t k = 0; k < order.size(); k++) {
    if (k % world != rank) continue;
    const uint32_t x0 = (order[k].second % tx) * tile, y0 = (order[k].second / tx) * tile;
    const uint32_t x1 = std::min(W, x0 + tile), y1 = std::min(H, y0 + tile);
    if (tilesOut) tilesOut->push_back({x0, y0, x1 - x0, y1 - y0, uint32_t(pixels.size()), (x1 - x0) * (y1 - y0)});
    for (uint32_t y = y0; y < y1; y++)
      for (uint32_t x = x0; x < x1; x++) pixels.push_back(x | (y << 16));
  }
  return pixels;
}
void buildPixelList(YartScene& s, uint32_t W, uint32_t H, uint32_t tile, uint32_t rank, uint32_t world) {
  if (s.pixW == W && s.pixH == H && s.pixTile == tile && s.pixRank == rank && s.pixWorld == world) return;
  s.pixelsHost = makePixelList(W, H, tile, rank, world, &s.tiles);
  s.pixels.upload(s.pixelsHost);
  {
    std::vector<uint32_t> start, count;
    for (const YartScene::TileRec& t : s.tiles) { start.push_back(t.start); count.push_back(t.count); }
    s.tileStart.upload(start); s.tileCount.upload(count);
  }
  s.pixW = W; s.pixH = H; s.pixTile = tile; s.pixRank = rank; s.pixWorld = world;
}

void validate(const YartCameraDesc* cam, const YartRenderParams* p) {
  require(cam && p, "camera / params pointer is null");
  require(cam->width > 0 && cam->height > 0 && cam->width < 65536 && cam->height < 65536,
          "image size must be in [1, 65535]");
  require(p->samples > 0 && p->first_wave_samples > 0 && p->max_wave_samples > 0, "sample counts must be > 0");
  require(p->tile_size > 0 && p->tile_size <= 4096, "tile_size out of range");
  require(p->shard_tile <= 4096, "shard_tile out of range");
  require(p->world_size > 0 && p->rank < p->world_size, "rank / world_size");
  require(p->max_depth > 0 && p->max_depth <= 255, "max_depth must be in [1, 255]");
  require(p->start_sample < p->samples && (p->stop_sample == 0 || (p->stop_sample > p->start_sample && p->stop_sample <= p->samples)),
          "start_sample / stop_sample out of range");
  require(p->estimator <= YART_ESTIMATOR_GMONB, "estimator must be one of YART_ESTIMATOR_*");
}

RenderConst makeRenderConst(const YartRenderParams& p) {
  RenderConst rc;
  rc.sampler = makeSamplerConfig(p.samples, p.tile_size);
  rc.maxDepth = p.max_depth;
  rc.background = mk3(p.background[0], p.background[1], p.background[2]);
  return rc;
}

int persistentGrid(const YartScene& s, const void* kernel, int cap, int block = kBlock) {
  int perCU = 0;
  HIP_CHECK(hipOccupancyMaxActiveBlocksPerMultiprocessor(&perCU, kernel, block, 0));
  if (perCU < 1) perCU = 1;
  if (perCU > cap) perCU = cap;
  return s.numCUs * perCU;
}

struct StageTimer {
  std::vector<hipEvent_t> ev;
  size_t used = 0;
  double ms = 0.0;
  uint32_t launches = 0;
  ~StageTimer() { for (auto e : ev) (void)hipEventDestroy(e); }
  hipEvent_t next() {
    if (used == ev.size()) { hipEvent_t e; HIP_CHECK(hipEventCreate(&e)); ev.push_back(e); }
    return ev[used++];
  }
  void begin(hipStream_t st) { HIP_CHECK(hipEventRecord(next(), st)); }
  void end(hipStream_t st) { HIP_CHECK(hipEventRecord(next(), st)); launches++; }
  void resolve() {
    for (size_t i = 0; i + 1 < used; i += 2) {
      float t = 0; HIP_CHECK(hipEventElapsedTime(&t, ev[i], ev[i + 1]));
      ms += t;
    }
    used = 0;
  }
};
struct StageTimers {
  StageTimer mega, extend, shade, connect, gmon, lean, shadeK, shadowLean;
  void resolveAll() { for (StageTimer* t : {&mega, &extend, &shade, &connect, &gmon, &lean, &shadeK, &shadowLean}) t->resolve(); }
};

struct BatchInfo { uint32_t c0, n, wave, waveSamples, samplesTaken, totalSamples; };
typedef std::function<bool(const BatchInfo&)> BatchHook;

struct RenderPlan {
  const YartRenderParams* p;
  const YartAovBuffers* aov;
  const YartMomentBuffers* mom;
  uint32_t W, H, nPix;
  CameraDev cam;
  RenderConst rc, rcw;
  uint32_t effFlags;
  bool mega, pool, compact, general, refill, samplerTables;
  int nodesForm;
  uint32_t nodeBitWords;
  void (*kMega)(MegaArgs);
  WfKernelFn kExtendFast, kShadowFast, kRetryE, kRetryS, kExtendGen, kExtendGenRetry, kShadowGen, kShadowGenRetry, kShade;
  int gridMega, gridExtendFast, gridShadowFast, gridExtend, gridShadow, gridShade, gridRetryE, gridRetryS, gridMax;
  uint32_t chunk, waveCap;
  size_t aovStride;
  size_t slots;
  uint32_t poolSlots, resumeCap;
};

struct BatchBudget { uint64_t maxPaths, poolFit; };
BatchBudget batchBudget(const YartScene& s, const RenderPlan& pl) {
  const YartRenderParams& p = *pl.p;
  const uint32_t nPix = pl.nPix;
  uint64_t maxPaths = p.max_batch_paths ? p.max_batch_paths : kDefaultBatchPaths;
  uint64_t poolFit = ~0ull;
  if (!pl.mega) {
    size_t freeB = 0, totalB = 0;
    HIP_CHECK(hipMemGetInfo(&freeB, &totalB));
    if (const char* e = std::getenv("YART_FAKE_FREE_MB")) freeB = size_t(std::max<long long>(1, std::atoll(e))) << 20;
    uint64_t held = uint64_t(s.L.n) * 16 + (uint64_t(s.qA.n) + s.qB.n + s.qS.n + s.qR.n) * 4 + uint64_t(s.resumeRec.n) * 16;
    for (auto& b : s.wf) held += uint64_t(b.n) * 16;
    for (auto& t : s.wfTail) for (auto& b : t) held += uint64_t(b.n) * 16;
    held += (uint64_t(s.wfTailMap[0].n) + s.wfTailMap[1].n) * 4;
    held += uint64_t(s.smpEntries.n) * 8;
    held += uint64_t(s.aovRec.n) * 16;
    if (std::getenv("YART_FAKE_FREE_MB")) held = 0;
    const uint64_t perPath = (pl.compact ? 251 : 176) + ((p.flags & YART_FLAG_NO_RESUME) ? 0 : (kResumeWords * 16 + 7) / 8);
    const uint64_t dimsEst = std::min<uint32_t>(256u, (4u + 8u * p.max_depth + 16u + 7u) & ~7u);
    const uint64_t fixedB = uint64_t(nPix) * dimsEst * 8 + uint64_t(pl.gridMax) * kBlock * (kResumeWords * 16 + uint64_t(spillDepthFor(s.host, true)) * 8) +
                            (pl.mom ? uint64_t(nPix) * sizeof(MomentState) : 0u);
    const uint64_t budget = (uint64_t(freeB) + held) * 8 / 10;
    const uint64_t avail = budget > fixedB ? budget - fixedB : 0;
    if (!pl.pool) {
      const uint64_t fits = std::max<uint64_t>(avail / perPath, 1u << 16);
      maxPaths = std::min<uint64_t>(std::min<uint64_t>(maxPaths, fits), kWfMaxPaths);
    } else {
      const uint64_t perBatchPath = pl.aov ? 16 + 48 : 16;
      const uint64_t fits = std::max<uint64_t>(avail / 2 / perBatchPath, 1u << 16);
      maxPaths = std::min<uint64_t>(maxPaths, fits);
      const uint64_t left = avail > std::min<uint64_t>(maxPaths, uint64_t(nPix ? nPix : 1) * pl.waveCap) * perBatchPath ? avail - std::min<uint64_t>(maxPaths, uint64_t(nPix ? nPix : 1) * pl.waveCap) * perBatchPath : 0;
      poolFit = std::max<uint64_t>(left / (176 + (kResumeWords * 16 + 7) / 8), 64);
    }
  }
  return {std::min<uint64_t>(maxPaths, (1ull << 31) - 64), poolFit};
}

RenderPlan makeRenderPlan(YartScene& s, const YartCameraDesc& camDesc, const YartRenderParams& p, const YartAovBuffers* aov,
                          const YartMomentBuffers* mom, hipStream_t stream) {
  RenderPlan pl{};
  pl.p = &p; pl.aov = aov; pl.mom = mom;
  pl.W = camDesc.width; pl.H = camDesc.height; pl.nPix = uint32_t(s.pixelsHost.size());
  pl.cam = makeCamera(camDesc);
  pl.rc = pl.rcw = makeRenderConst(p);
  pl.mega = (p.flags & YART_FLAG_MEGAKERNEL) != 0;
  pl.effFlags = p.flags;
  if (!pl.mega && !(pl.effFlags & YART_FLAG_NO_SHADE_SORT)) pl.effFlags |= YART_FLAG_SHADE_SORT;

  pl.general = (p.flags & YART_FLAG_GENERAL_TRACE) != 0;
  const bool ident = s.host.allIdentity;
  pl.refill = (p.flags & YART_FLAG_NO_REFILL) == 0;
  const bool chunked = s.host.nodes.size() >= 64;
  const bool tlasOk = s.dev.nTlas != 0u && s.host.nodes.size() <= 16384u && !(pl.effFlags & (262144u | 65536u));
  const bool leanLds = !chunked && s.host.nodes.size() <= kLeanSceneNodes && s.host.meshes.size() <= kLeanSceneNodes;
  pl.nodesForm = !chunked ? (leanLds ? kNodesMaskLds : kNodesMask) : tlasOk ? kNodesTlas
               : ((pl.effFlags & 65536u) || s.host.nodes.size() >= kLeanWalkNodes) ? kNodesWalk : kNodesChunked;
  pl.kExtendFast = wfKernel(pl.refill ? tu::extendLean(pl.nodesForm, ident) : tu::extendFast(ident));
  pl.kShadowFast = wfKernel(pl.refill ? tu::shadowLean(pl.nodesForm, ident) : tu::shadowFast(ident));
  pl.kRetryE = wfKernel(tu::extendRetry(pl.nodesForm));
  pl.kRetryS = wfKernel(tu::shadowRetry(pl.nodesForm));
  pl.kExtendGen = wfKernel(tu::extendGeneral(false)); pl.kExtendGenRetry = wfKernel(tu::extendGeneral(true));
  pl.kShadowGen = wfKernel(tu::shadowGeneral(false)); pl.kShadowGenRetry = wfKernel(tu::shadowGeneral(true));
  pl.kMega = aov ? k_render_mega<true> : k_render_mega<false>;
  pl.gridMega = persistentGrid(s, reinterpret_cast<const void*>(pl.kMega), 3);
  pl.gridExtendFast = persistentGrid(s, reinterpret_cast<const void*>(pl.kExtendFast), 8);
  pl.gridShadowFast = persistentGrid(s, reinterpret_cast<const void*>(pl.kShadowFast), 8);
  pl.gridExtend = persistentGrid(s, reinterpret_cast<const void*>(pl.kExtendGen), 8);
  pl.gridShadow = persistentGrid(s, reinterpret_cast<const void*>(pl.kShadowGen), 8);
  pl.samplerTables = !pl.mega && !(p.flags & YART_FLAG_DIRECT_SAMPLER) && pl.nPix > 0 && uint64_t(p.samples) <= (1ull << pl.rc.sampler.log2spp);
  const bool shadeFit = pl.samplerTables && s.dev.nMaterials <= kShadeMatSlots && s.dev.nTextures <= kShadeTexSlots && s.dev.nLights <= kShadeLightSlots &&
                        s.dev.nEnvs <= kShadeEnvSlots && s.dev.nNodes <= kShadeNodeSlots && s.dev.nInfinite <= kShadeLightSlots;
  const bool envOnly = shadeFit && s.dev.nArea == 0u && s.dev.nInfinite == 1u && s.dev.nLights == 1u;
  pl.kShade = wfKernel(tu::shade((pl.effFlags & YART_FLAG_SHADE_SORT) != 0, shadeFit, envOnly));
  pl.gridShade = persistentGrid(s, reinterpret_cast<const void*>(pl.kShade), 8, kShadeBlock);
  pl.gridRetryE = persistentGrid(s, reinterpret_cast<const void*>(pl.kRetryE), 8);
  pl.gridRetryS = persistentGrid(s, reinterpret_cast<const void*>(pl.kRetryS), 8);
  pl.gridMax = std::max(pl.gridMega, std::max(pl.gridExtend, pl.gridShadow));
  pl.gridMax = std::max(pl.gridMax, std::max(pl.gridExtendFast, pl.gridShadowFast));
  pl.gridMax = std::max(pl.gridMax, std::max(pl.gridRetryE, pl.gridRetryS));
  s.spill.ensure(size_t(pl.gridMax) * kBlock * spillDepthFor(s.host, true));
  pl.nodeBitWords = pl.nodesForm == kNodesTlas ? uint32_t((s.host.nodes.size() + 63u) / 64u) : 0u;
  if (pl.nodeBitWords) {
    const size_t need = size_t(pl.gridMax) * kBlock * pl.nodeBitWords;
    if (s.nodeBits.n < need) { s.nodeBits.ensure(need); HIP_CHECK(hipMemsetAsync(s.nodeBits.p, 0, need * 8, stream)); }
  }

  const uint32_t maxWave = std::min(p.max_wave_samples, p.samples);
  pl.waveCap = std::max(std::min(p.first_wave_samples, p.samples), maxWave);
  pl.pool = !pl.mega && (p.flags & YART_FLAG_PATH_POOL) != 0;
  pl.compact = !pl.mega && !pl.pool && !(p.flags & YART_FLAG_NO_COMPACTION);
  const BatchBudget fit = batchBudget(s, pl);
  pl.chunk = uint32_t(std::min<uint64_t>(pl.nPix ? pl.nPix : 1, std::max<uint64_t>(fit.maxPaths / pl.waveCap, 1)));
  if (pl.nPix > pl.chunk) {
    const uint32_t nb = (pl.nPix + pl.chunk - 1) / pl.chunk;
    pl.chunk = (pl.nPix + nb - 1) / nb;
  }
  pl.aovStride = size_t(pl.chunk) * pl.waveCap;
  if (!pl.mega) {
    pl.slots = pl.aovStride;
    if (pl.pool) {
      const size_t want = std::min<uint64_t>(p.pool_paths ? p.pool_paths : kDefaultPoolPaths, fit.poolFit);
      pl.slots = std::max<size_t>(64, (std::min(want, pl.aovStride) + 63) & ~size_t(63));
      pl.poolSlots = uint32_t(pl.slots);
    }
    if (!(p.flags & YART_FLAG_NO_RESUME)) {
      size_t cap = std::max<size_t>(pl.slots / 8, std::min<size_t>(pl.slots, 1u << 16)) + size_t(pl.gridMax) * kBlock;
      if (const char* e = std::getenv("YART_RESUME_CAP")) cap = size_t(std::max<long long>(0, std::atoll(e)));
      pl.resumeCap = uint32_t(std::min<size_t>(cap, 0x7fffff00u));
    }
  }
  return pl;
}

void prepareBuffers(YartScene& s, const RenderPlan& pl, hipStream_t stream) {
  const size_t np1 = std::max<uint32_t>(pl.nPix, 1u), wh = size_t(pl.W) * pl.H;
  const auto clear = [&](void* ptr, int byte, size_t bytes) { HIP_CHECK(hipMemsetAsync(ptr, byte, bytes, stream)); };
  s.L.ensure(pl.aovStride);
  if (pl.aov) {
    for (auto& b : s.aovAcc) { b.ensure(np1); clear(b.p, 0, np1 * sizeof(f4)); }
    s.aovRays.ensure(np1); clear(s.aovRays.p, 0, np1 * sizeof(uint32_t));
    s.aovIds.ensure(np1 * 4); clear(s.aovIds.p, 0xff, np1 * 4 * sizeof(int32_t));
    s.pixRays.ensure(np1);
    if (pl.mega || pl.pool) s.aovRec.ensure(3 * pl.aovStride);
    clearBuffers(kAovTable, *pl.aov, wh, clear);
  }
  if (pl.mom) {
    s.momState.ensure(np1); clear(s.momState.p, 0, np1 * sizeof(MomentState));
    clearBuffers(kMomentTable, *pl.mom, wh, clear);
  }
  if (pl.mega) return;
  if (pl.pool) {
    s.poolMap.ensure(pl.slots);
    if (!s.poolHost) HIP_CHECK(hipHostMalloc(reinterpret_cast<void**>(&s.poolHost), kPoolLag * WC_COUNT * sizeof(uint32_t)));
  }
  for (auto& b : s.wf) b.ensure(pl.slots);
  if (pl.compact) {
    for (auto& b : s.wfTail[0]) b.ensure(pl.slots / 2 + 64);
    s.wfTailMap[0].ensure(pl.slots / 2 + 64);
    s.wfTailMap[1].ensure(pl.slots / 4 + 64);
    s.wfDyn.ensure(1);
  }
  s.qA.ensure(pl.slots); s.qB.ensure(pl.slots); s.qS.ensure(pl.slots); s.qR.ensure(pl.slots); s.wfCounters.ensure(WC_COUNT);
  if (pl.resumeCap) s.resumeRec.ensure(size_t(pl.resumeCap) * kResumeWords);
}

void launchSamplerTables(YartScene& s, RenderPlan& pl, StageTimers& t, hipStream_t stream) {
  if (!pl.samplerTables) return;
  const uint32_t dims = std::min<uint32_t>(256u, (4u + 8u * pl.p->max_depth + 16u + 7u) & ~7u);
  s.smpEntries.ensure(size_t(dims) * pl.nPix); s.smpHash.ensure(dims + 3); s.smpSobol1.ensure(8 * 256);
  SamplerTabArgs ta{};
  ta.cfg = pl.rc.sampler; ta.pixels = s.pixels.p; ta.nPixels = pl.nPix; ta.dims = dims;
  ta.entries = s.smpEntries.p; ta.hash = s.smpHash.p; ta.sobol1 = s.smpSobol1.p;
  ta.matrix52 = reinterpret_cast<const uint32_t*>(s.dev.lut + LutDev::sobol);
  TraceRange rg("yart:sampler_tables", stream);
  t.shade.begin(stream);
  hipLaunchKernelGGL(k_sampler_tables, dim3(s.numCUs * 8), dim3(kBlock), 0, stream, ta);
  HIP_CHECK(hipGetLastError());
  t.shade.end(stream);
  pl.rcw.sampler.tab.entries = s.smpEntries.p; pl.rcw.sampler.tab.hash = s.smpHash.p; pl.rcw.sampler.tab.sobol1 = s.smpSobol1.p;
  pl.rcw.sampler.tab.dims = dims; pl.rcw.sampler.tab.stride = pl.nPix;
}

struct Batch { uint32_t c0, n, waveSamples, takenBefore; };

AovArgs aovArgs(const YartScene& s, const RenderPlan& pl, const Batch& b) {
  AovArgs av{};
  if (pl.aov) {
    av.acc0 = s.aovAcc[0].p; av.acc1 = s.aovAcc[1].p; av.acc2 = s.aovAcc[2].p; av.accRays = s.aovRays.p; av.ids = s.aovIds.p;
    av.nPixels = b.n; av.spp = b.waveSamples; av.pixBase = b.c0; av.sampleOffset = b.takenBefore;
    if (pl.mega || pl.pool) { av.r0 = s.aovRec.p; av.r1 = s.aovRec.p + pl.aovStride; av.r2 = s.aovRec.p + 2 * pl.aovStride; }
  }
  return av;
}
void aovReduce(const AovArgs& av, hipStream_t stream) {
  TraceRange rgA("yart:aov_reduce", stream);
  hipLaunchKernelGGL(k_aov_reduce, dim3((av.nPixels * 4u + kBlock - 1) / kBlock), dim3(kBlock), 0, stream, av);
  HIP_CHECK(hipGetLastError());
}

void runMegaBatch(YartScene& s, const RenderPlan& pl, const Batch& b, StageTimers& t, hipStream_t stream) {
  const AovArgs av = aovArgs(s, pl, b);
  HIP_CHECK(hipMemsetAsync(s.cursor.p, 0, sizeof(uint32_t), stream));
  MegaArgs a{};
  a.sc = s.dev; a.cam = pl.cam; a.rc = pl.rc; a.pixels = s.pixels.p + b.c0; a.nPixels = b.n;
  a.spp = b.waveSamples; a.sampleOffset = b.takenBefore; a.L = s.L.p;
  a.cursor = s.cursor.p; a.rays = s.counters.p; a.spill = s.spill.p;
  a.aov0 = av.r0; a.aov1 = av.r1; a.aov2 = av.r2; a.aovIds = av.ids; a.pixBase = b.c0;
  TraceRange rgMega("yart:megakernel", stream);
  t.mega.begin(stream);
  hipLaunchKernelGGL(pl.kMega, dim3(pl.gridMega), dim3(kBlock), 0, stream, a);
  HIP_CHECK(hipGetLastError());
  t.mega.end(stream);
  if (pl.aov) aovReduce(av, stream);
}

WfArgs wfArgs(const YartScene& s, const RenderPlan& pl, const Batch& b) {
  WfArgs a{};
  a.sc = s.dev; a.cam = pl.cam; a.rc = pl.rcw; a.pixBase = b.c0;
  a.st.ray0 = s.wf[0].p; a.st.ray1 = s.wf[1].p; a.st.thr = s.wf[2].p; a.st.acc = s.wf[3].p;
  a.st.hit0 = s.wf[4].p; a.st.hit1 = s.wf[5].p; a.st.sh0 = s.wf[6].p; a.st.sh1 = s.wf[7].p; a.st.sh2 = s.wf[8].p;
  a.qA = s.qA.p; a.qB = s.qB.p; a.qS = s.qS.p; a.qR = s.qR.p; a.counters = s.wfCounters.p;
  a.pixels = s.pixels.p + b.c0; a.nPaths = b.n * b.waveSamples; a.spp = b.waveSamples;
  a.sampleOffset = b.takenBefore; a.L = s.L.p; a.stats = s.counters.p; a.spill = s.spill.p;
  a.matClass = s.matClass.p;
  a.resumeRec = pl.resumeCap ? s.resumeRec.p : nullptr; a.resumeCap = pl.resumeCap;
  a.sc.nodeBits = s.nodeBits.p; a.sc.nodeBitWords = pl.nodeBitWords;
  return a;
}

void extendStage(const RenderPlan& pl, const WfArgs& a, StageTimers& t, hipStream_t stream) {
  t.extend.begin(stream);
  if (pl.general) {
    hipLaunchKernelGGL(pl.kExtendGen, dim3(pl.gridExtend), dim3(kBlock), 0, stream, a);
  } else {
    t.lean.begin(stream);
    hipLaunchKernelGGL(pl.kExtendFast, dim3(pl.gridExtendFast), dim3(kBlock), 0, stream, a);
    t.lean.end(stream);
    if (pl.refill) hipLaunchKernelGGL(pl.kRetryE, dim3(pl.gridRetryE), dim3(kBlock), 0, stream, a);
    else hipLaunchKernelGGL(pl.kExtendGenRetry, dim3(pl.gridExtend), dim3(kBlock), 0, stream, a);
    hipLaunchKernelGGL(k_wf_reset_retry, dim3(1), dim3(64), 0, stream, a.counters);
  }
  HIP_CHECK(hipGetLastError());
  t.extend.end(stream);
}
void shadowStage(const RenderPlan& pl, const WfArgs& a, StageTimers& t, hipStream_t stream) {
  t.connect.begin(stream);
  if (pl.general) {
    hipLaunchKernelGGL(pl.kShadowGen, dim3(pl.gridShadow), dim3(kBlock), 0, stream, a);
  } else {
    t.shadowLean.begin(stream);
    hipLaunchKernelGGL(pl.kShadowFast, dim3(pl.gridShadowFast), dim3(kBlock), 0, stream, a);
    t.shadowLean.end(stream);
    if (pl.refill) hipLaunchKernelGGL(pl.kRetryS, dim3(pl.gridRetryS), dim3(kBlock), 0, stream, a);
    else hipLaunchKernelGGL(pl.kShadowGenRetry, dim3(pl.gridShadow), dim3(kBlock), 0, stream, a);
  }
  HIP_CHECK(hipGetLastError());
  t.connect.end(stream);
}
void shadeStage(const RenderPlan& pl, const WfArgs& a, StageTimers& t, hipStream_t stream) {
  t.shade.begin(stream);
  t.shadeK.begin(stream);
  hipLaunchKernelGGL(pl.kShade, dim3(pl.gridShade), dim3(kShadeBlock), 0, stream, a);
  HIP_CHECK(hipGetLastError());
  t.shadeK.end(stream);
  t.shade.end(stream);
}
void streamingPass(const YartScene& s, WfKernelFn k, const WfArgs& a, StageTimers& t, hipStream_t stream) {
  t.shade.begin(stream);
  hipLaunchKernelGGL(k, dim3(s.numCUs * YART_STREAM_BLOCKS), dim3(kBlock), 0, stream, a);
  HIP_CHECK(hipGetLastError());
  t.shade.end(stream);
}

void runPoolBatch(YartScene& s, const RenderPlan& pl, const Batch& b, StageTimers& t, hipStream_t stream) {
  const AovArgs av = aovArgs(s, pl, b);
  WfArgs a = wfArgs(s, pl, b);
  a.slotMap = s.poolMap.p;
  a.poolSlots = uint32_t(std::min<uint64_t>(pl.poolSlots, (uint64_t(a.nPaths) + 63u) & ~uint64_t(63)));
  const uint32_t init[WC_COUNT] = {a.poolSlots, 0, 0, 0, 0, 0, 0, 0, 0, 0};
  HIP_CHECK(hipMemcpyAsync(s.wfCounters.p, init, sizeof(init), hipMemcpyHostToDevice, stream));
  hipLaunchKernelGGL(k_wf_pool_init, dim3(s.numCUs * 4), dim3(kBlock), 0, stream, s.poolMap.p, a.poolSlots);
  HIP_CHECK(hipGetLastError());
  struct RoundEvents {
    hipEvent_t ev[kPoolLag] = {};
    ~RoundEvents() { for (auto e : ev) if (e) (void)hipEventDestroy(e); }
  } roundEv;
  hipEvent_t* evRound = roundEv.ev;
  for (int k = 0; k < kPoolLag; k++) HIP_CHECK(hipEventCreateWithFlags(&evRound[k], hipEventDisableTiming));
  const uint64_t maxRounds = (uint64_t(a.nPaths) / a.poolSlots + 2u) * (pl.rc.maxDepth + 1u) + 16u;
  bool done = false;
  for (uint64_t round = 0; !done; round++) {
    if (round > maxRounds) throw HipError("path pool: the batch did not finish within its bound of rounds");
    streamingPass(s, k_wf_refill, a, t, stream);
    {
      uint32_t* snap = s.poolHost + size_t(round % kPoolLag) * WC_COUNT;
      HIP_CHECK(hipMemcpyAsync(snap, s.wfCounters.p, WC_COUNT * sizeof(uint32_t), hipMemcpyDeviceToHost, stream));
      HIP_CHECK(hipEventRecord(evRound[round % kPoolLag], stream));
    }
    extendStage(pl, a, t, stream);
    if (pl.aov) {
      hipLaunchKernelGGL(k_aov_capture, dim3(s.numCUs * YART_STREAM_BLOCKS), dim3(kBlock), 0, stream, a, av);
      HIP_CHECK(hipGetLastError());
    }
    shadeStage(pl, a, t, stream);
    shadowStage(pl, a, t, stream);
    streamingPass(s, k_wf_roulette, a, t, stream);
    hipLaunchKernelGGL(k_wf_pool_advance, dim3(1), dim3(64), 0, stream, s.wfCounters.p, a.poolSlots);
    HIP_CHECK(hipGetLastError());
    if (round >= 2) {
      const uint64_t old = round - 2;
      HIP_CHECK(hipEventSynchronize(evRound[old % kPoolLag]));
      const uint32_t* c = s.poolHost + size_t(old % kPoolLag) * WC_COUNT;
      if (c[WC_NEXT] == 0u) done = true;
    }
  }
  if (pl.aov) aovReduce(av, stream);
}

void runWavefrontBatch(YartScene& s, const RenderPlan& pl, const Batch& b, StageTimers& t, hipStream_t stream) {
  AovArgs av = aovArgs(s, pl, b);
  WfArgs a = wfArgs(s, pl, b);
  const uint32_t maxDepth = pl.rc.maxDepth;
  if (pl.compact) {
    for (int k = 0; k < 2; k++) {
      f4** f = &a.tail[k].ray0;
      for (int j = 0; j < 9; j++) f[j] = k == 0 ? s.wfTail[0][j].p : s.wf[j].p;
      a.tailMap[k] = s.wfTailMap[k].p;
      a.tailCap[k] = a.nPaths / (k == 0 ? 2u : 4u);
    }
    WfDyn d0{};
    d0.st = a.st; d0.slotMap = nullptr; d0.extent = a.nPaths; d0.inTail = 0;
    HIP_CHECK(hipMemcpyAsync(s.wfDyn.p, &d0, sizeof(d0), hipMemcpyHostToDevice, stream));
    a.dyn = s.wfDyn.p;
  }
  const uint32_t init[WC_COUNT] = {a.nPaths, 0, 0, 0, 0, 0, 0, 0, 0};
  HIP_CHECK(hipMemcpyAsync(s.wfCounters.p, init, sizeof(init), hipMemcpyHostToDevice, stream));
  {
    TraceRange rgGen("yart:generate", stream);
    streamingPass(s, k_wf_generate, a, t, stream);
  }
  for (uint32_t bounce = 0; bounce < maxDepth; bounce++) {
    a.bounce = bounce;
    char rgName[32]; std::snprintf(rgName, sizeof(rgName), "yart:bounce %u", bounce);
    TraceRange rgBounce(rgName);
    {
      TraceRange rgExtend("yart:extend", stream);
      extendStage(pl, a, t, stream);
    }
    if (pl.aov && bounce == 0) {
      {
        TraceRange rgA("yart:aov_capture", stream);
        av.r0 = a.st.sh0; av.r1 = a.st.sh1; av.r2 = a.st.sh2;
        hipLaunchKernelGGL(k_aov_capture, dim3(s.numCUs * YART_STREAM_BLOCKS), dim3(kBlock), 0, stream, a, av);
        HIP_CHECK(hipGetLastError());
      }
      aovReduce(av, stream);
    }
    {
      TraceRange rgShade("yart:shade", stream);
      shadeStage(pl, a, t, stream);
    }
    {
      TraceRange rgShadow("yart:shadow", stream);
      shadowStage(pl, a, t, stream);
    }
    const bool thinning = bounce >= 1 && bounce + 1 < maxDepth;
    if (thinning) { TraceRange rgR("yart:roulette"); }
    hipLaunchKernelGGL(k_wf_advance, dim3(1), dim3(64), 0, stream, s.wfCounters.p, bounce + 1 < 16u ? s.pathsLog.p + bounce + 1 : nullptr);
    HIP_CHECK(hipGetLastError());
    std::swap(a.qA, a.qB);
    if (pl.compact && thinning) {
      TraceRange rgC("yart:compact", stream);
      t.shade.begin(stream);
      hipLaunchKernelGGL(k_wf_compact, dim3(s.numCUs * YART_STREAM_BLOCKS), dim3(kBlock), 0, stream, a);
      hipLaunchKernelGGL(k_wf_compact_commit, dim3(1), dim3(64), 0, stream, a);
      HIP_CHECK(hipGetLastError());
      t.shade.end(stream);
    }
  }
}

struct WaveInfo { uint32_t wave, samplesTaken; float wCurrent, wWave; size_t tileDone; };
bool finishBatch(YartScene& s, const RenderPlan& pl, const Batch& b, WaveInfo& w, float* dOut, StageTimers& t, const BatchHook* hook,
                 hipStream_t stream) {
  const uint32_t c0 = b.c0, n = b.n;
  const bool hooked = hook && *hook;
  GmonArgs g{};
  if (hooked) { s.pixRays.ensure(std::max<uint32_t>(pl.nPix, 1u)); g.pixRays = s.pixRays.p + c0; }
  if (pl.aov) g.pixRays = s.pixRays.p + c0;
  g.L = s.L.p; g.pixels = s.pixels.p + c0; g.nPixels = n; g.spp = b.waveSamples; g.width = pl.W;
  g.exposureScale = pl.cam.exposureScale; g.wCurrent = w.wCurrent; g.wWave = w.wWave; g.hdr = dOut;
  g.kind = int(pl.p->estimator);
  {
    TraceRange rgBlend("yart:gmon_blend", stream);
    t.gmon.begin(stream);
    hipLaunchKernelGGL(k_gmon_blend, dim3((n + kGmonPixPerBlock - 1) / kGmonPixPerBlock), dim3(kBlock), 0, stream, g);
    HIP_CHECK(hipGetLastError());
    t.gmon.end(stream);
    if (pl.mom) {
      MomentArgs ma{};
      ma.L = s.L.p; ma.state = s.momState.p; ma.nPixels = n; ma.spp = b.waveSamples; ma.pixBase = c0;
      ma.exposureScale = pl.cam.exposureScale;
      TraceRange rgM("yart:moments_accumulate", stream);
      hipLaunchKernelGGL(k_moments_accumulate, dim3((n + kMomentPixPerBlock - 1) / kMomentPixPerBlock), dim3(kBlock), 0, stream, ma);
      HIP_CHECK(hipGetLastError());
    }
    if (pl.aov) {
      hipLaunchKernelGGL(k_aov_add_rays, dim3((n + kBlock - 1) / kBlock), dim3(kBlock), 0, stream, s.aovRays.p + c0, s.pixRays.p + c0, n);
      HIP_CHECK(hipGetLastError());
    }
    HIP_CHECK(hipStreamSynchronize(stream));
  }
  t.resolveAll();
  if (!hooked) return false;
  size_t done = w.tileDone;
  while (done < s.tiles.size() && s.tiles[done].start + s.tiles[done].count <= c0 + n) done++;
  if (done > w.tileDone) {
    s.tileRays.ensure(s.tiles.size()); s.tileRaysHost.resize(s.tiles.size());
    hipLaunchKernelGGL(k_tile_rays, dim3(uint32_t(done - w.tileDone)), dim3(64), 0, stream, s.pixRays.p, s.tileStart.p, s.tileCount.p,
                       uint32_t(w.tileDone), uint32_t(done - w.tileDone), s.tileRays.p);
    HIP_CHECK(hipGetLastError());
    HIP_CHECK(hipMemcpyAsync(s.tileRaysHost.data() + w.tileDone, s.tileRays.p + w.tileDone, (done - w.tileDone) * sizeof(unsigned long long),
                             hipMemcpyDeviceToHost, stream));
    HIP_CHECK(hipStreamSynchronize(stream));
    w.tileDone = done;
  }
  return (*hook)(BatchInfo{c0, n, w.wave, b.waveSamples, w.samplesTaken, pl.p->samples});
}

void launchFinishKernels(const YartScene& s, const RenderPlan& pl, hipStream_t stream) {
  if (pl.nPix == 0) return;
  if (pl.aov) {
    const YartAovBuffers* aov = pl.aov;
    AovFinishArgs f{};
    f.acc0 = s.aovAcc[0].p; f.acc1 = s.aovAcc[1].p; f.acc2 = s.aovAcc[2].p; f.accRays = s.aovRays.p; f.ids = s.aovIds.p;
    f.pixels = s.pixels.p; f.nPixels = pl.nPix; f.width = pl.W; f.samples = pl.p->samples; f.mask = aov->mask;
    f.albedo = aov->albedo; f.normal = aov->normal; f.position = aov->position; f.depth = aov->depth; f.coverage = aov->coverage;
    f.outIds = aov->ids; f.outRays = aov->rays;
    TraceRange rgA("yart:aov_finish", stream);
    hipLaunchKernelGGL(k_aov_finish, dim3((pl.nPix + kBlock - 1) / kBlock), dim3(kBlock), 0, stream, f);
    HIP_CHECK(hipGetLastError());
  }
  if (pl.mom) {
    const YartMomentBuffers* mom = pl.mom;
    MomentFinishArgs f{};
    f.state = s.momState.p; f.pixels = s.pixels.p; f.nPixels = pl.nPix; f.width = pl.W; f.mask = mom->mask;
    f.mean = mom->mean; f.variance = mom->variance; f.count = mom->count;
    TraceRange rgM("yart:moments_finish", stream);
    hipLaunchKernelGGL(k_moments_finish, dim3((pl.nPix + kBlock - 1) / kBlock), dim3(kBlock), 0, stream, f);
    HIP_CHECK(hipGetLastError());
  }
}

YartStats makeStats(const YartScene& s, const RenderPlan& pl, const StageTimers& t, const unsigned long long* cnt, float msAll,
                    uint32_t waves, uint64_t renderedSamples) {
  YartStats st{};
  st.samples = uint64_t(pl.nPix) * renderedSamples;
  st.rays = cnt[0];
  st.traversals = cnt[1]; st.box_tests = cnt[2]; st.tri_tests = cnt[3]; st.shaded_hits = cnt[4];
  st.ms_device = msAll;
  st.ms_traverse = pl.mega ? t.mega.ms : t.extend.ms + t.connect.ms;
  st.launches_traverse = pl.mega ? t.mega.launches : t.extend.launches + t.connect.launches;
  st.ms_extend = t.extend.ms; st.ms_shade = t.shade.ms; st.ms_connect = t.connect.ms; st.ms_gmon = t.gmon.ms;
  st.ms_extend_lean = t.lean.ms; st.launches_extend_lean = t.lean.launches;
  st.lean_traversals = cnt[5]; st.lean_box_tests = cnt[6]; st.lean_tri_tests = cnt[7];
  st.ms_shade_kernel = t.shadeK.ms; st.launches_shade_kernel = t.shadeK.launches;
  st.ms_shadow_lean = t.shadowLean.ms; st.launches_shadow_lean = t.shadowLean.launches;
  st.shadow_lean_traversals = cnt[24]; st.shadow_lean_box_tests = cnt[25]; st.shadow_lean_tri_tests = cnt[26];
  st.shade_entries = cnt[28]; st.retry_extend_traversals = cnt[29]; st.retry_shadow_traversals = cnt[30];
  st.pipeline_flags = pl.effFlags;
  {
    unsigned long long paths[16] = {0};
    HIP_CHECK(hipMemcpy(paths, s.pathsLog.p, sizeof(paths), hipMemcpyDeviceToHost));
    for (int b = 0; b < 16; b++) st.paths_at_bounce[b] = paths[b];
    st.paths_at_bounce[0] = pl.mega || pl.pool ? 0 : uint64_t(pl.nPix) * renderedSamples;
  }
#if defined(YART_COUNT_TRAVERSAL)
  {
    unsigned long long tb = 0;
    HIP_CHECK(hipMemcpyFromSymbol(&tb, HIP_SYMBOL(g_texTapBytes), sizeof(tb)));
    tb += tu::texTapRead1() + tu::texTapRead2() + tu::texTapRead3() + tu::texTapRead4();
    st.texture_tap_bytes = tb;
  }
#endif
  st.launches_extend = t.extend.launches; st.launches_connect = t.connect.launches;
  st.waves = waves;
  return st;
}

bool renderToDevice(YartScene& s, const YartCameraDesc& camDesc, const YartRenderParams& p, float* dOut,
                    hipStream_t stream, YartStats* stats, const BatchHook* hook = nullptr, const YartAovBuffers* aov = nullptr,
                    const YartMomentBuffers* mom = nullptr) {
  bool aborted = false;
  auto wall0 = std::chrono::high_resolution_clock::now();
  TraceRange rgRender("yart:render");
  HIP_CHECK(hipSetDevice(s.device));
  buildPixelList(s, camDesc.width, camDesc.height, p.shard_tile ? p.shard_tile : p.tile_size, p.rank, p.world_size);
  const uint64_t startSample = p.start_sample, stopSample = p.stop_sample ? p.stop_sample : p.samples;
  if (startSample == 0) HIP_CHECK(hipMemsetAsync(dOut, 0, size_t(camDesc.width) * camDesc.height * 4 * sizeof(float), stream));
  s.cursor.ensure(1); s.counters.ensure(kNumCounters); s.pathsLog.ensure(16);
  HIP_CHECK(hipMemsetAsync(s.pathsLog.p, 0, 16 * sizeof(unsigned long long), stream));
  HIP_CHECK(hipMemsetAsync(s.counters.p, 0, kNumCounters * sizeof(unsigned long long), stream));
#if defined(YART_COUNT_TRAVERSAL)
  { const unsigned long long zero = 0; HIP_CHECK(hipMemcpyToSymbol(HIP_SYMBOL(g_texTapBytes), &zero, sizeof(zero))); tu::texTapReset1(); tu::texTapReset2(); tu::texTapReset3(); tu::texTapReset4(); }
#endif
  RenderPlan pl = makeRenderPlan(s, camDesc, p, aov, mom, stream);
  prepareBuffers(s, pl, stream);

  Timer tAll;
  StageTimers t;
  uint32_t waves = 0;
  uint64_t renderedSamples = 0;
  HIP_CHECK(hipEventRecord(tAll.a, stream));
  launchSamplerTables(s, pl, t, stream);
  const auto runBatch = pl.mega ? runMegaBatch : pl.pool ? runPoolBatch : runWavefrontBatch;

  for (WaveSchedule ws(p.samples, p.first_wave_samples, p.max_wave_samples); !aborted && ws.next();) {
    const bool inRange = ws.takenBefore >= startSample && ws.takenBefore < stopSample;
    if (!inRange && ws.takenBefore < startSample && ws.takenAfter > startSample) throw std::invalid_argument("start_sample is not a wave boundary");
    if (inRange && ws.takenAfter > stopSample) throw std::invalid_argument("stop_sample is not a wave boundary");
    if (!inRange) continue;
    waves++; renderedSamples += ws.samples;
    WaveInfo w{uint32_t(ws.wave), uint32_t(ws.takenAfter), float(ws.takenBefore) / float(ws.takenAfter), float(ws.samples) / float(ws.takenAfter), 0};
    for (uint32_t c0 = 0; !aborted && c0 < pl.nPix; c0 += pl.chunk) {
      const Batch b{c0, std::min(pl.chunk, pl.nPix - c0), uint32_t(ws.samples), uint32_t(ws.takenBefore)};
      runBatch(s, pl, b, t, stream);
      aborted = finishBatch(s, pl, b, w, dOut, t, hook, stream);
    }
  }
  if (!aborted) launchFinishKernels(s, pl, stream);
  HIP_CHECK(hipEventRecord(tAll.b, stream));
  HIP_CHECK(hipEventSynchronize(tAll.b));
  float msAll = 0; HIP_CHECK(hipEventElapsedTime(&msAll, tAll.a, tAll.b));
  unsigned long long cnt[kNumCounters] = {0};
  HIP_CHECK(hipMemcpy(cnt, s.counters.p, sizeof(cnt), hipMemcpyDeviceToHost));
  for (int i = 0; i < kNumCounters; i++) s.lastCounters[i] = cnt[i];
  if (stats) {
    *stats = makeStats(s, pl, t, cnt, msAll, waves, renderedSamples);
    stats->ms_total = std::chrono::duration<double, std::milli>(std::chrono::high_resolution_clock::now() - wall0).count();
  }
  return aborted;
}

struct RcclFailure : std::runtime_error { using std::runtime_error::runtime_error; };

template <class F>
int guarded(F&& f) {
  try {
    f();
    return YART_OK;
  } catch (const RcclFailure& e) {
    g_lastError = e.what(); return YART_E_RCCL;
  } catch (const std::invalid_argument& e) {
    g_lastError = e.what(); return YART_E_INVALID;
  } catch (const HipError& e) {
    g_lastError = e.what();
    int count = 0;
    if (hipGetDeviceCount(&count) != hipSuccess || count <= 0) return YART_E_NO_DEVICE;
    return YART_E_HIP;
  } catch (const std::exception& e) {
    g_lastError = e.what(); return YART_E_IO;
  }
}

}

namespace {
std::unique_ptr<LoadedScene> importGltf(const char* path, const YartImportOptions* opts) {
  auto loaded = gltf::loadGltf(path);
  if (opts) {
    const float radius = opts->env_radius > 0.0f ? opts->env_radius : 100.0f;
    if (opts->env_hdr_path && opts->env_hdr_path[0]) gltf::addImageEnvironment(*loaded, opts->env_hdr_path, radius);
    if (opts->uniform_env) gltf::addUniformEnvironment(*loaded, opts->uniform_emission, radius);
  }
  return loaded;
}
}

#include "multi_device.inc"

extern "C" {

int yart_hip_abi_version(void) { return YART_HIP_ABI_VERSION; }

int yart_hip_device_count(void) {
  int count = 0;
  if (hipGetDeviceCount(&count) != hipSuccess) return 0;
  return count;
}

const char* yart_hip_last_error(void) { return g_lastError.c_str(); }

int yart_hip_scene_create(const YartSceneDesc* desc, int device, YartScene** out) {
  return guarded([&] {
    require(desc && out, "desc / out pointer is null");
    *out = createScene(*desc, device);
  });
}

int yart_hip_scene_create_flags(const YartSceneDesc* desc, int device, uint32_t scene_flags, YartScene** out) {
  return guarded([&] {
    require(desc && out, "desc / out pointer is null");
    *out = createScene(*desc, device, scene_flags);
  });
}

int yart_hip_scene_load(const char* path, int device, YartScene** out) {
  return guarded([&] {
    require(path && out, "path / out pointer is null");
    auto loaded = loadSceneFile(path);
    *out = createScene(loaded->desc, device);
  });
}

int yart_hip_scene_load_gltf(const char* path, const YartImportOptions* opts, int device, YartScene** out) {
  return guarded([&] {
    require(path && out, "path / out pointer is null");
    auto loaded = importGltf(path, opts);
    *out = createScene(loaded->desc, device);
  });
}

int yart_hip_gltf_to_yscn(const char* gltf_path, const YartImportOptions* opts, const char* yscn_path) {
  return guarded([&] {
    require(gltf_path && yscn_path, "path pointer is null");
    auto loaded = importGltf(gltf_path, opts);
    saveSceneFile(loaded->desc, yscn_path);
  });
}

void yart_hip_scene_destroy(YartScene* scene) {
  if (!scene) return;
  (void)hipSetDevice(scene->device);
  delete scene;
}

int yart_hip_render_device(YartScene* scene, const YartCameraDesc* cam, const YartRenderParams* params,
                           float* d_out_rgba, void* stream, YartStats* stats) {
  return guarded([&] {
    require(scene && d_out_rgba, "scene / output pointer is null");
    validate(cam, params);
    std::lock_guard<std::mutex> lock(scene->mu);
    renderToDevice(*scene, *cam, *params, d_out_rgba, static_cast<hipStream_t>(stream), stats);
  });
}

int yart_hip_render(YartScene* scene, const YartCameraDesc* cam, const YartRenderParams* params,
                    float* out_rgba, YartStats* stats) {
  return guarded([&] {
    require(scene && out_rgba, "scene / output pointer is null");
    validate(cam, params);
    std::lock_guard<std::mutex> lock(scene->mu);
    auto t0 = std::chrono::high_resolution_clock::now();
    HIP_CHECK(hipSetDevice(scene->device));
    const size_t n = size_t(cam->width) * cam->height * 4;
    scene->hdr.ensure(n);
    if (params->start_sample > 0) HIP_CHECK(hipMemcpy(scene->hdr.p, out_rgba, n * sizeof(float), hipMemcpyHostToDevice));
    renderToDevice(*scene, *cam, *params, scene->hdr.p, nullptr, stats);
    HIP_CHECK(hipMemcpy(out_rgba, scene->hdr.p, n * sizeof(float), hipMemcpyDeviceToHost));
    if (stats)
      stats->ms_total = std::chrono::duration<double, std::milli>(std::chrono::high_resolution_clock::now() - t0).count();
  });
}

static bool checkAovs(const YartAovBuffers* in, const YartCameraDesc* cam, const YartRenderParams* params, YartAovBuffers& out) {
  out = YartAovBuffers{};
  if (in) checkAndCopyBuffers(kAovTable, *in, out);
  validate(cam, params);
  if (out.mask != 0u)
    require(params->start_sample == 0 && (params->stop_sample == 0 || params->stop_sample == params->samples),
            "feature buffers need the full sample range (start_sample = 0, stop_sample = 0 or samples)");
  return out.mask != 0u;
}

static bool checkMoments(const YartMomentBuffers* in, const YartRenderParams* params, YartMomentBuffers& out) {
  out = YartMomentBuffers{};
  if (in) checkAndCopyBuffers(kMomentTable, *in, out);
  if (out.mask != 0u && params)
    require(params->start_sample == 0 && (params->stop_sample == 0 || params->stop_sample == params->samples),
            "sample moments need the full sample range (start_sample = 0, stop_sample = 0 or samples)");
  return out.mask != 0u;
}

int yart_hip_render_moments_device(YartScene* scene, const YartCameraDesc* cam, const YartRenderParams* params, float* d_out_rgba,
                                   const YartAovBuffers* d_aovs, const YartMomentBuffers* d_moments, void* stream, YartStats* stats) {
  return guarded([&] {
    YartAovBuffers av;
    YartMomentBuffers mv;
    const bool any = checkAovs(d_aovs, cam, params, av);
    const bool anyM = checkMoments(d_moments, params, mv);
    require(scene && d_out_rgba, "scene / output pointer is null");
    std::lock_guard<std::mutex> lock(scene->mu);
    renderToDevice(*scene, *cam, *params, d_out_rgba, static_cast<hipStream_t>(stream), stats, nullptr, any ? &av : nullptr,
                   anyM ? &mv : nullptr);
  });
}

int yart_hip_render_aovs_device(YartScene* scene, const YartCameraDesc* cam, const YartRenderParams* params, float* d_out_rgba,
                                const YartAovBuffers* d_aovs, void* stream, YartStats* stats) {
  return yart_hip_render_moments_device(scene, cam, params, d_out_rgba, d_aovs, nullptr, stream, stats);
}

int yart_hip_render_moments(YartScene* scene, const YartCameraDesc* cam, const YartRenderParams* params, float* out_rgba,
                            const YartAovBuffers* aovs, const YartMomentBuffers* moments, YartStats* stats) {
  return guarded([&] {
    YartAovBuffers host;
    YartMomentBuffers hostM;
    const bool any = checkAovs(aovs, cam, params, host);
    const bool anyM = checkMoments(moments, params, hostM);
    require(scene && out_rgba, "scene / output pointer is null");
    std::lock_guard<std::mutex> lock(scene->mu);
    auto t0 = std::chrono::high_resolution_clock::now();
    HIP_CHECK(hipSetDevice(scene->device));
    const size_t wh = size_t(cam->width) * cam->height, n = wh * 4;
    scene->hdr.ensure(n);
    if (params->start_sample > 0) HIP_CHECK(hipMemcpy(scene->hdr.p, out_rgba, n * sizeof(float), hipMemcpyHostToDevice));
    YartAovBuffers dev = host;
    if (any) {
      scene->aovOut.ensure(layOutBuffers(kAovTable, host.mask, wh, nullptr, dev));
      layOutBuffers(kAovTable, host.mask, wh, scene->aovOut.p, dev);
    }
    YartMomentBuffers devM = hostM;
    if (anyM) {
      scene->momOut.ensure(layOutBuffers(kMomentTable, hostM.mask, wh, nullptr, devM));
      layOutBuffers(kMomentTable, hostM.mask, wh, scene->momOut.p, devM);
    }
    renderToDevice(*scene, *cam, *params, scene->hdr.p, nullptr, stats, nullptr, any ? &dev : nullptr, anyM ? &devM : nullptr);
    HIP_CHECK(hipMemcpy(out_rgba, scene->hdr.p, n * sizeof(float), hipMemcpyDeviceToHost));
    const auto toHost = [](void* dst, const void* src, size_t bytes) { HIP_CHECK(hipMemcpy(dst, src, bytes, hipMemcpyDeviceToHost)); };
    if (any) copyBuffers(kAovTable, host, dev, wh, toHost);
    if (anyM) copyBuffers(kMomentTable, hostM, devM, wh, toHost);
    if (stats)
      stats->ms_total = std::chrono::duration<double, std::milli>(std::chrono::high_resolution_clock::now() - t0).count();
  });
}

int yart_hip_render_aovs(YartScene* scene, const YartCameraDesc* cam, const YartRenderParams* params, float* out_rgba,
                         const YartAovBuffers* aovs, YartStats* stats) {
  return yart_hip_render_moments(scene, cam, params, out_rgba, aovs, nullptr, stats);
}

static int renderProgressive(YartScene* scene, const YartCameraDesc* cam, const YartRenderParams* params, float* out_rgba,
                             YartStats* stats, YartWaveCallback on_wave, YartTileCallback on_tile, void* user) {
  bool aborted = false;
  const int rc = guarded([&] {
    require(scene && out_rgba, "scene / output pointer is null");
    validate(cam, params);
    std::lock_guard<std::mutex> lock(scene->mu);
    auto t0 = std::chrono::high_resolution_clock::now();
    HIP_CHECK(hipSetDevice(scene->device));
    const uint32_t W = cam->width, H = cam->height;
    const size_t n = size_t(W) * H * 4;
    scene->hdr.ensure(n);
    const uint32_t stop = params->stop_sample ? params->stop_sample : params->samples;
    if (params->start_sample > 0) HIP_CHECK(hipMemcpy(scene->hdr.p, out_rgba, n * sizeof(float), hipMemcpyHostToDevice));
    else if (on_tile) std::memset(out_rgba, 0, n * sizeof(float));
    YartStats total{};
    for (WaveSchedule ws(params->samples, params->first_wave_samples, params->max_wave_samples); !aborted && ws.next();) {
      const uint32_t taken = uint32_t(ws.takenBefore);
      const uint64_t wave = ws.wave, waveSamples = ws.samples;
      if (taken >= params->start_sample && taken < stop) {
        YartRenderParams q = *params;
        q.start_sample = taken; q.stop_sample = uint32_t(taken + waveSamples);
        YartStats st{};
        auto tw = std::chrono::high_resolution_clock::now();
        size_t nextTile = 0;
        BatchHook hook = [&](const BatchInfo& b) {
          const auto& tiles = scene->tiles;
          bool stopNow = false;
          while (nextTile < tiles.size() && tiles[nextTile].start + tiles[nextTile].count <= b.c0 + b.n) {
            const YartScene::TileRec& t = tiles[nextTile++];
            const size_t off = (size_t(t.y) * W + t.x) * 4;
            HIP_CHECK(hipMemcpy2D(out_rgba + off, size_t(W) * 16, scene->hdr.p + off, size_t(W) * 16, size_t(t.w) * 16, t.h,
                                  hipMemcpyDeviceToHost));
            YartTileInfo ti{};
            ti.x = t.x; ti.y = t.y; ti.width = t.w; ti.height = t.h;
            ti.index = uint32_t(nextTile); ti.total = uint32_t(tiles.size());
            ti.wave = b.wave; ti.wave_samples = b.waveSamples; ti.samples_taken = b.samplesTaken; ti.total_samples = b.totalSamples;
            ti.rays = nextTile - 1 < scene->tileRaysHost.size() ? scene->tileRaysHost[nextTile - 1] : 0;
            ti.ms = std::chrono::duration<double, std::milli>(std::chrono::high_resolution_clock::now() - tw).count();
            if (on_tile(user, &ti) != 0) stopNow = true;
          }
          return stopNow;
        };
        const bool stopped = renderToDevice(*scene, *cam, q, scene->hdr.p, nullptr, &st, on_tile ? &hook : nullptr);
        if (!on_tile || stopped) HIP_CHECK(hipMemcpy(out_rgba, scene->hdr.p, n * sizeof(float), hipMemcpyDeviceToHost));
        total.rays += st.rays; total.waves += st.waves; total.ms_device += st.ms_device; total.samples += st.samples;
        total.ms_extend += st.ms_extend; total.ms_shade += st.ms_shade; total.ms_connect += st.ms_connect; total.ms_gmon += st.ms_gmon;
        total.ms_traverse += st.ms_traverse; total.launches_traverse += st.launches_traverse;
        total.pipeline_flags = st.pipeline_flags;
        st.ms_total = std::chrono::duration<double, std::milli>(std::chrono::high_resolution_clock::now() - t0).count();
        if (stopped) aborted = true;
        else if (on_wave && on_wave(user, &st, uint32_t(wave), uint32_t(waveSamples), uint32_t(taken + waveSamples), params->samples) != 0)
          aborted = true;
      }
    }
    total.ms_total = std::chrono::duration<double, std::milli>(std::chrono::high_resolution_clock::now() - t0).count();
    if (stats) *stats = total;
  });
  return rc == YART_OK && aborted ? YART_ABORTED : rc;
}

int yart_hip_render_waves(YartScene* scene, const YartCameraDesc* cam, const YartRenderParams* params,
                          float* out_rgba, YartStats* stats, YartWaveCallback on_wave, void* user) {
  return renderProgressive(scene, cam, params, out_rgba, stats, on_wave, nullptr, user);
}

int yart_hip_render_tiles(YartScene* scene, const YartCameraDesc* cam, const YartRenderParams* params,
                          float* out_rgba, YartStats* stats, YartWaveCallback on_wave, YartTileCallback on_tile, void* user) {
  return renderProgressive(scene, cam, params, out_rgba, stats, on_wave, on_tile, user);
}

int yart_hip_multi_create(const YartSceneDesc* desc, const int* devices, uint32_t n_devices, YartMulti** out) {
  return guarded([&] {
    require(desc && out, "desc / out pointer is null");
    *out = createMulti(*desc, devices, n_devices);
  });
}

int yart_hip_multi_load(const char* path, const YartImportOptions* opts, const int* devices, uint32_t n_devices, YartMulti** out) {
  return guarded([&] {
    require(path && out, "path / out pointer is null");
    const std::string p(path);
    const bool gltf = p.size() > 4 && (p.rfind(".glb") == p.size() - 4 || p.rfind(".gltf") == p.size() - 5);
    auto loaded = gltf ? importGltf(path, opts) : loadSceneFile(path);
    *out = createMulti(loaded->desc, devices, n_devices);
  });
}

void yart_hip_multi_destroy(YartMulti* multi) { delete multi; }

int yart_hip_multi_rccl_selftest(int device, uint32_t n_floats) {
  return guarded([&] {
    require(n_floats > 0 && n_floats <= (1u << 26), "n_floats out of range");
    const int dev = resolveDevice(device);
    if (dev < 0) throw HipError("no usable HIP device (libyart_hip has no CPU fallback)");
    HIP_CHECK(hipSetDevice(dev));
    const RcclApi& R = rccl();
    ncclComm_t comm = nullptr;
    RCCL_CHECK(R.CommInitAll(&comm, 1, &dev));
    hipStream_t st = nullptr;
    DevBuf<float> a, b;
    std::vector<float> h(n_floats), back(n_floats, 0.0f);
    for (uint32_t i = 0; i < n_floats; i++) h[i] = float(i % 8191u) * 0.25f - 3.0f;
    try {
      HIP_CHECK(hipStreamCreate(&st));
      a.upload(h); b.ensure(n_floats);
      HIP_CHECK(hipMemsetAsync(b.p, 0, size_t(n_floats) * 4, st));
      RCCL_CHECK(R.GroupStart());
      ncclResult_t e = R.Send(a.p, n_floats, ncclFloat, 0, comm, st);
      if (e == ncclSuccess) e = R.Recv(b.p, n_floats, ncclFloat, 0, comm, st);
      const ncclResult_t ge = R.GroupEnd();
      RCCL_CHECK(e);
      RCCL_CHECK(ge);
      HIP_CHECK(hipStreamSynchronize(st));
      HIP_CHECK(hipMemcpy(back.data(), b.p, size_t(n_floats) * 4, hipMemcpyDeviceToHost));
    } catch (...) {
      if (st) (void)hipStreamDestroy(st);
      (void)R.CommDestroy(comm);
      throw;
    }
    (void)hipStreamDestroy(st);
    RCCL_CHECK(R.CommDestroy(comm));
    if (std::memcmp(h.data(), back.data(), size_t(n_floats) * 4) != 0) throw RcclFailure("rccl selftest: the received slab differs from the sent one");
  });
}

int yart_hip_multi_device_count(const YartMulti* multi) { return multi ? int(multi->scenes.size()) : 0; }

int yart_hip_multi_failed_devices(const YartMulti* multi, int* replicas_out, uint32_t capacity) {
  if (!multi) return 0;
  int nf = 0;
  for (size_t i = 0; i < multi->failed.size(); i++)
    if (multi->failed[i]) { if (replicas_out && uint32_t(nf) < capacity) replicas_out[nf] = int(i); nf++; }
  if (nf) g_lastError = multi->failureNote;
  return nf;
}

int yart_hip_multi_render(YartMulti* multi, const YartCameraDesc* cam, const YartRenderParams* params, float* out_rgba,
                          YartStats* stats) {
  return guarded([&] {
    require(multi && out_rgba, "multi / output pointer is null");
    validate(cam, params);
    renderMulti(*multi, *cam, *params, out_rgba, stats);
  });
}

int yart_hip_multi_render_tiles(YartMulti* multi, const YartCameraDesc* cam, const YartRenderParams* params, float* out_rgba,
                                YartStats* stats, YartWaveCallback on_wave, YartTileCallback on_tile, void* user) {
  bool aborted = false;
  const int rc = guarded([&] {
    require(multi && out_rgba, "multi / output pointer is null");
    validate(cam, params);
    aborted = renderMultiProgressive(*multi, *cam, *params, out_rgba, stats, on_wave, on_tile, user) == YART_ABORTED;
  });
  return rc == YART_OK && aborted ? YART_ABORTED : rc;
}

int yart_hip_debug_counters(YartScene* scene, uint64_t* out32) {
  return guarded([&] {
    require(scene && out32, "null pointer");
    for (int i = 0; i < kNumCounters; i++) out32[i] = scene->lastCounters[i];
  });
}

int yart_hip_debug_shade_regions(uint64_t* out48) {
#if defined(YART_SHADE_REGIONS)
  return guarded([&] {
    require(out48 != nullptr, "null pointer");
    unsigned long long v[3 * 16];
    tu::shadeRegionsTake(v);
    for (int i = 0; i < 48; i++) out48[i] = v[i];
  });
#else
  (void)out48;
  return YART_E_INVALID;
#endif
}

int yart_hip_bvh_info(YartScene* scene, uint32_t mesh, uint32_t* n_nodes, uint32_t* n_tris) {
  return guarded([&] {
    require(scene && n_nodes && n_tris, "null pointer");
    require(mesh < scene->host.meshes.size(), "mesh index out of range");
    *n_nodes = scene->host.meshes[mesh].nNodes;
    *n_tris = scene->host.meshes[mesh].nTris;
  });
}

int yart_hip_bvh_copy(YartScene* scene, uint32_t mesh, uint32_t* nodes_out, uint32_t* indices_out) {
  return guarded([&] {
    require(scene && nodes_out && indices_out, "null pointer");
    require(mesh < scene->host.meshes.size(), "mesh index out of range");
    const MeshDev& m = scene->host.meshes[mesh];
    HIP_CHECK(hipSetDevice(scene->device));
    HIP_CHECK(hipMemcpy(nodes_out, scene->bvhNodes.p + m.nodeOffset, size_t(m.nNodes) * sizeof(BvhNode),
                        hipMemcpyDeviceToHost));
    for (uint32_t n = 0; n < m.nNodes; n++) nodes_out[size_t(n) * 8 + 6] &= kLinkIndexMask;
    std::memcpy(indices_out, scene->host.bvhIndices[mesh].data(), size_t(m.nTris) * 4);
  });
}

static void checkBvhBuildArgs(const float* positions, uint32_t n_verts, const uint32_t* faces, uint32_t face_stride, uint32_t n_faces,
                              const uint32_t* nodes_out, const uint32_t* indices_out, const uint32_t* n_nodes) {
  require(positions && faces && nodes_out && indices_out && n_nodes, "null pointer");
  require(n_faces >= 1 && n_faces <= kLinkIndexMask && face_stride >= 3, "bvh build: bad triangle count or stride");
  for (size_t k = 0; k < size_t(n_faces) * face_stride; k += face_stride)
    for (int c = 0; c < 3; c++) require(faces[k + c] < n_verts, "bvh build: vertex index out of range");
}

int yart_hip_bvh_build_device(int device, const float* positions, uint32_t n_verts, const uint32_t* faces, uint32_t face_stride,
                              uint32_t n_faces, uint32_t* nodes_out, uint32_t* indices_out, uint32_t* n_nodes, double* ms_device) {
  return guarded([&] {
    checkBvhBuildArgs(positions, n_verts, faces, face_stride, n_faces, nodes_out, indices_out, n_nodes);
    std::vector<BvhNode> nodes;
    std::vector<uint32_t> indices;
    require(devbvh::build(device, positions, n_verts, faces, face_stride, n_faces, nodes, indices, ms_device),
            "bvh build: refused on the device (NaN coordinate or tree deeper than 192 levels): build on the host");
    *n_nodes = uint32_t(nodes.size());
    std::memcpy(nodes_out, nodes.data(), nodes.size() * sizeof(BvhNode));
    std::memcpy(indices_out, indices.data(), indices.size() * 4);
  });
}

int yart_hip_bvh_build_host(const float* positions, uint32_t n_verts, const uint32_t* faces, uint32_t face_stride, uint32_t n_faces,
                            uint32_t threads, uint32_t* nodes_out, uint32_t* indices_out, uint32_t* n_nodes, double* ms_host) {
  return guarded([&] {
    checkBvhBuildArgs(positions, n_verts, faces, face_stride, n_faces, nodes_out, indices_out, n_nodes);
    const auto t0 = std::chrono::steady_clock::now();
    SahBvhBuilder b;
    b.setThreads(threads);
    b.build(positions, faces, face_stride, n_faces);
    if (ms_host) *ms_host = std::chrono::duration<double, std::milli>(std::chrono::steady_clock::now() - t0).count();
    *n_nodes = uint32_t(b.nodes.size());
    std::memcpy(nodes_out, b.nodes.data(), b.nodes.size() * sizeof(BvhNode));
    std::memcpy(indices_out, b.indices.data(), b.indices.size() * 4);
  });
}

}

#include "postprocess.inc"
#include "scene_update_kernels.inc"
#include "mesh_update_kernels.inc"
#include "probes.inc"
```

Before: 676.5 Msamples/s.

## Replace separate compaction pass with in-shade migration into per-bounce arena regions

Removes the standalone compact kernel, which copied the surviving path state into tail buffers, and the dynamic state indirection (WfDyn) that it required. Instead, the shade kernel allocates wave-sized chunks in a per-bounce region of a single enlarged arena through an atomic bump counter and writes surviving paths directly into it, updating the slot map. Russian roulette is also decided inside shade before migration, so dead paths are never written. This avoids a full extra read and write of the survivor state each bounce and a kernel launch, at the cost of extra atomics and LDS coordination in shade, a larger arena, and more complex shade code.

```diff
diff --git a/yart_amd/csrc/region_plan.hpp b/yart_amd/csrc/region_plan.hpp
--- /dev/null
+++ b/yart_amd/csrc/region_plan.hpp
@@ -0,0 +1,68 @@
+#pragma once
+#include <cstdint>
+
+namespace yart_hip {
+
+#if defined(__HIPCC__)
+#define YART_RP_HD __host__ __device__ inline
+#else
+#define YART_RP_HD inline
+#endif
+
+constexpr uint32_t kMaxRegions = 4;
+#ifndef YART_REGIONS
+#define YART_REGIONS 4
+#endif
+constexpr uint32_t kRegionAsk = 64;
+constexpr uint32_t kRegionRangeMax = 1024;
+
+struct RegionPlan {
+  uint32_t k;
+  uint32_t off[kMaxRegions];
+  uint32_t cap[kMaxRegions];
+  uint64_t end;
+};
+YART_RP_HD RegionPlan makeRegionPlan(uint32_t nPaths, uint32_t k, uint32_t capDiv = 1u) {
+  RegionPlan p{};
+  p.k = k > kMaxRegions ? kMaxRegions : k;
+  uint64_t at = (uint64_t(nPaths) + 63u) & ~uint64_t(63);
+  for (uint32_t r = 0; r < p.k; r++) {
+    const uint32_t want = (nPaths >> (r + 1u)) / (capDiv ? capDiv : 1u);
+    p.off[r] = uint32_t(at);
+    p.cap[r] = want < 64u ? 64u : ((want + 63u) & ~63u);
+    at += p.cap[r];
+  }
+  p.end = at;
+  return p;
+}
+YART_RP_HD bool regionPlanFits(const RegionPlan& p) { return p.end < (1ull << 31); }
+YART_RP_HD uint64_t regionBytesPerPath(uint32_t k) {
+  uint64_t b = 148u * 16u;
+  for (uint32_t r = 0; r < k && r < kMaxRegions; r++) b += (148u * 16u) >> (r + 1u);
+  return (b + 15u) / 16u;
+}
+
+YART_RP_HD uint32_t regionRange(uint32_t count, uint32_t nWaves) {
+  const uint32_t per = nWaves != 0u ? nWaves * 4u : 1u;
+  const uint32_t c = (count / per) & ~15u;
+  return c > kRegionRangeMax ? kRegionRangeMax : c;
+}
+
+struct RegionRange { uint32_t cur, end; };
+constexpr uint32_t kRegionNone = 0xffffffffu;
+struct RegionTake { uint32_t first, nFirst, second; };
+YART_RP_HD uint32_t regionSlot(const RegionTake& t, uint32_t k) { return k < t.nFirst ? t.first + k : t.second + (k - t.nFirst); }
+template <class Bump>
+YART_RP_HD RegionTake regionAsk(RegionRange& r, uint32_t n, uint32_t range, uint32_t cap, Bump&& bump) {
+  RegionTake t{kRegionNone, 0u, 0u};
+  const uint32_t left = r.end - r.cur;
+  if (left >= n) { t.first = r.cur; t.nFirst = n; r.cur += n; return t; }
+  const uint32_t size = range > n - left ? range : n - left;
+  const uint32_t old = bump(size);
+  if (old == kRegionNone || uint64_t(old) + size > cap) return t;
+  t.first = r.cur; t.nFirst = left; t.second = old;
+  r.cur = old + (n - left); r.end = old + size;
+  return t;
+}
+
+}
diff --git a/yart_amd/csrc/stream_kernels.inc b/yart_amd/csrc/stream_kernels.inc
--- a/yart_amd/csrc/stream_kernels.inc
+++ b/yart_amd/csrc/stream_kernels.inc
@@ -23,7 +23,6 @@
 }
 
 __global__ void __launch_bounds__(kBlock) k_wf_generate(WfArgs a) {
-  WF_DYN(a);
   const uint32_t* sobol = reinterpret_cast<const uint32_t*>(a.sc.lut + LutDev::sobol);
   __shared__ SamplerLds smpLds;
   samplerToLds(a.rc.sampler, smpLds, true);
@@ -32,6 +31,7 @@
     const uint32_t pk = a.pixels[pi];
     wfGenerate(a.rc, sobol, a.cam, pk & 0xffffu, pk >> 16, s + a.sampleOffset, a.pixBase + pi, a.st, i);
     a.qA[i] = i;
+    if (a.slotMap) a.slotMap[i] = i;
   }
 }
 
@@ -88,59 +88,16 @@
   if (threadIdx.x == 0 && blockIdx.x == 0) { counters[WC_RETRY] = 0; counters[WC_CUR_RETRY] = 0; counters[WC_RESUME] = 0; }
 }
 
-#ifndef YART_COMPACT_NUM
-#define YART_COMPACT_NUM 1
-#define YART_COMPACT_DEN 2
-#endif
-__device__ __forceinline__ bool wfCompactPlan(const WfArgs& a, const WfDyn& d, uint32_t count, uint32_t& dst) {
-  dst = d.inTail == 1u ? 1u : 0u;
-  return count > 0u && count <= a.tailCap[dst] && uint64_t(YART_COMPACT_DEN) * count <= uint64_t(YART_COMPACT_NUM) * d.extent;
-}
-__global__ void __launch_bounds__(kBlock) k_wf_compact(WfArgs a) {
-  const WfDyn d = *a.dyn;
-  const uint32_t count = a.counters[WC_ACTIVE];
-  uint32_t dst;
-  if (!wfCompactPlan(a, d, count, dst)) return;
-  const WfState from = d.st, to = a.tail[dst];
-  uint32_t* map = a.tailMap[dst];
-  const uint32_t stride = gridDim.x * blockDim.x;
-  for (uint32_t k0 = blockIdx.x * blockDim.x + threadIdx.x; k0 < count; k0 += 2u * stride) {
-    const uint32_t k1 = k0 + stride;
-    const bool v1 = k1 < count;
-    const uint32_t s0 = a.qA[k0], s1 = v1 ? a.qA[k1] : s0;
-    const f4 a0 = wfLd(from.ray0 + s0), b0 = wfLd(from.ray1 + s0), c0 = wfLd(from.thr + s0), d0 = wfLd(from.acc + s0), e0 = wfLd(from.hit1 + s0);
-    const f4 a1 = wfLd(from.ray0 + s1), b1 = wfLd(from.ray1 + s1), c1 = wfLd(from.thr + s1), d1 = wfLd(from.acc + s1), e1 = wfLd(from.hit1 + s1);
-    const uint32_t m0 = d.slotMap ? d.slotMap[s0] : s0, m1 = d.slotMap ? d.slotMap[s1] : s1;
-    wfSt(to.ray0 + k0, a0); wfSt(to.ray1 + k0, b0); wfSt(to.thr + k0, c0); wfSt(to.acc + k0, d0); wfSt(to.hit1 + k0, e0);
-    map[k0] = m0; a.qA[k0] = k0;
-    if (v1) {
-      wfSt(to.ray0 + k1, a1); wfSt(to.ray1 + k1, b1); wfSt(to.thr + k1, c1); wfSt(to.acc + k1, d1); wfSt(to.hit1 + k1, e1);
-      map[k1] = m1; a.qA[k1] = k1;
-    }
-  }
-}
-__global__ void k_wf_compact_commit(WfArgs a) {
-  if (threadIdx.x != 0 || blockIdx.x != 0) return;
-  const WfDyn d = *a.dyn;
-  const uint32_t count = a.counters[WC_ACTIVE];
-  uint32_t dst;
-  if (!wfCompactPlan(a, d, count, dst)) return;
-  WfDyn n;
-  n.st = a.tail[dst]; n.slotMap = a.tailMap[dst]; n.extent = count; n.inTail = dst + 1u;
-  *a.dyn = n;
-}
-
 __global__ void k_wf_advance(uint32_t* counters, unsigned long long* pathsLog) {
   if (threadIdx.x == 0 && blockIdx.x == 0) {
     counters[0] = counters[1];
     if (pathsLog) *pathsLog += counters[1] - counters[WC_DUMMY];
-    for (uint32_t k = 1; k < WC_COUNT; k++) if (k != WC_STARTED) counters[k] = 0;
+    for (uint32_t k = 1; k < WC_REGION; k++) if (k != WC_STARTED) counters[k] = 0;
   }
 }
 
 __global__ void __launch_bounds__(kBlock) k_wf_roulette(WfArgs a) {
   WF_EMPTY_BLOCK(a.counters[WC_SHADOW], kBlock);
-  WF_DYN(a);
   const uint32_t count = a.counters[WC_SHADOW];
   const uint32_t stride = gridDim.x * blockDim.x;
   const uint32_t rounds = (count + stride - 1) / stride;
diff --git a/yart_amd/csrc/wavefront.hpp b/yart_amd/csrc/wavefront.hpp
--- a/yart_amd/csrc/wavefront.hpp
+++ b/yart_amd/csrc/wavefront.hpp
@@ -1,5 +1,6 @@
 #pragma once
 #include "integrator.hpp"
+#include "region_plan.hpp"
 
 namespace yart_hip {
 
@@ -290,11 +291,15 @@
   return true;
 }
 
-enum WfShadeResult { WF_TERMINATED = 0, WF_CONTINUE = 1, WF_SHADOW = 2, WF_SKIPPED = 3 };
-
+enum WfShadeResult { WF_TERMINATED = 0, WF_CONTINUE = 1, WF_SHADOW = 2, WF_SKIPPED = 3, WF_TERMINATED_RR = 4 };
+
+struct WfNext { uint32_t w, mapWord; bool toNext, moved; };
+
+template <class Migrate>
 YART_HD WfShadeResult wfShade(const SceneDev& sc, const RenderConst& rc, const uint32_t* sobol, const WfState& s,
-                              uint32_t i, WfPath& p, uint32_t& rays, WfTally& tally) {
+                              uint32_t i, WfPath& p, uint32_t& rays, WfTally& tally, bool pool, Migrate& mig, WfNext& nx) {
   p = wfLoad(s, i);
+  nx.w = i; nx.mapWord = 0; nx.toNext = false; nx.moved = false;
   if (p.flags & WF_DEAD) return WF_SKIPPED;
   if (p.flags & WF_RR_PENDING) wfRouletteScale(p.att);
   const f4 h0 = wfLd(s.hit0 + i);
@@ -355,17 +360,35 @@
   const f3 fcos = res.f * absDot(res.wi, hit.n);
   f3 newAtt = p.att * (fcos / res.pdf);
   if (hit.backSide) newAtt *= matAttenuation(mt, hit.t);
+  const bool nee = !(res.scatter & (SC_EMITTED | SC_SPECULAR));
+  const uint32_t depth1 = depth + 1u;
+  const bool rrApplies = depth1 > 1u && depth1 < rc.maxDepth && maxComponent(newAtt) < 1.0f;
+  bool rrDrawn = false, rrDies = false;
+  if (rrApplies && !pool) {
+    Sampler smpRr = p.smp;
+    if (nee && sc.nLights != 0) smpRr.dim += 3u;
+    const float q = stdmax(0.0f, 1.0f - maxComponent(newAtt));
+    rrDies = get1D(smpRr, rc.sampler) < q;
+    rrDrawn = true;
+  }
+  const bool goesOn = depth1 < rc.maxDepth && !rrDies;
+  const uint32_t w = mig.take(goesOn, i);
+  if (w != i) {
+    wfSt(s.hit1 + w, mk4(asF(nodeBack), asF(uint32_t(p.smp.morton)), asF(uint32_t(p.smp.morton >> 32)), asF(p.smp.pix)));
+    nx.mapWord = mig.map[i];
+    nx.moved = true;
+  }
+  nx.w = w;
   {
     WfPath q;
     q.o = hit.p; q.d = res.wi; q.lastPdf = res.pdf; q.accRoughness = p.accRoughness + res.roughness;
-    wfStoreRay(s, i, q);
-    uint32_t fl = ((depth + 1) & WF_DEPTH_MASK) | (p.flags & WF_NEE_MASK);
+    wfStoreRay(s, w, q);
+    uint32_t fl = (depth1 & WF_DEPTH_MASK) | (p.flags & WF_NEE_MASK);
     if (res.scatter & SC_SPECULAR) fl |= WF_SPECULAR;
     if (q.accRoughness > 0.5f) fl |= WF_REGULARIZED;
     p.flags = fl;
   }
   SR_MARK(6);
-  const bool nee = !(res.scatter & (SC_EMITTED | SC_SPECULAR));
 
   bool shadow = false;
   if (nee) {
@@ -388,9 +411,9 @@
         float pdfLight = pl * ls.pdf / absDot(ls.n, ls.wi);
         if (l.type == LIGHT_AREA) pdfLight *= length2(hit.p - ls.p);
         const f3 Lif = ls.Li * f;
-        wfSt(s.sh0 + i, mk4(ls.p.x, ls.p.y, ls.p.z, asF(p.smp.dim)));
-        wfSt(s.sh1 + i, mk4(p.att.x, p.att.y, p.att.z, pdfBSDF + pdfLight));
-        wfSt(s.sh2 + i, mk4(Lif.x, Lif.y, Lif.z, absDot(ls.wi, hit.n)));
+        wfSt(s.sh0 + w, mk4(ls.p.x, ls.p.y, ls.p.z, asF(p.smp.dim)));
+        wfSt(s.sh1 + w, mk4(p.att.x, p.att.y, p.att.z, pdfBSDF + pdfLight));
+        wfSt(s.sh2 + w, mk4(Lif.x, Lif.y, Lif.z, absDot(ls.wi, hit.n)));
         shadow = true;
         if ((p.flags & WF_DEPTH_MASK) >= rc.maxDepth) p.flags |= WF_FINAL;
         {
@@ -403,7 +426,21 @@
     if (!shadow) p.L += p.att * mk3(0.0f);
   }
   p.att = newAtt;
-  return shadow ? WF_SHADOW : WF_CONTINUE;
-}
-
-}
+  if (pool && !shadow && depth1 > 1u && maxComponent(p.att) < 1.0f) {
+    const float q = stdmax(0.0f, 1.0f - maxComponent(p.att));
+    if (get1D(p.smp, rc.sampler) < q) return WF_TERMINATED_RR;
+    p.att /= 1.0f - q;
+    nx.toNext = depth1 < rc.maxDepth;
+    return nx.toNext ? WF_CONTINUE : WF_TERMINATED_RR;
+  }
+  if (rrDrawn) {
+    p.smp.dim++;
+    if (shadow) { p.flags |= WF_RR_PENDING; if (rrDies) p.flags |= WF_FINAL; }
+    else if (!rrDies) { const float q = stdmax(0.0f, 1.0f - maxComponent(p.att)); p.att /= 1.0f - q; }
+  }
+  nx.toNext = goesOn && !(pool && shadow && depth1 > 1u);
+  if (shadow) return WF_SHADOW;
+  return goesOn ? WF_CONTINUE : WF_TERMINATED_RR;
+}
+
+}
diff --git a/yart_amd/csrc/wavefront_kernels.inc b/yart_amd/csrc/wavefront_kernels.inc
--- a/yart_amd/csrc/wavefront_kernels.inc
+++ b/yart_amd/csrc/wavefront_kernels.inc
@@ -13,22 +13,14 @@
 #define YART_WF_MAX_PATHS_LOG2 30
 #endif
 constexpr uint32_t kWfMaxPaths = 1u << YART_WF_MAX_PATHS_LOG2;
-
-struct WfDyn {
-  WfState st;
-  uint32_t* slotMap;
-  uint32_t extent;
-  uint32_t inTail;
-};
+static_assert(2ull * kWfMaxPaths - (kWfMaxPaths >> kMaxRegions) + 64ull * (kMaxRegions + 1u) < (1ull << 31), "arena of kWfMaxPaths paths");
+
 struct WfArgs {
   SceneDev sc;
   CameraDev cam;
   RenderConst rc;
-  WfDyn* dyn;
   uint32_t* slotMap;
-  WfState tail[2];
-  uint32_t* tailMap[2];
-  uint32_t tailCap[2];
+  uint32_t migOff, migCap, migRegion, padM;
   WfState st;
   uint32_t* qA;
   uint32_t* qB;
@@ -53,11 +45,11 @@
   WC_RESUME = 8,
   WC_STARTED = 9,
   WC_DUMMY = 10,
-  WC_COUNT = 11
+  WC_REGION = 11,
+  WC_COUNT = WC_REGION + kMaxRegions
 };
 
 #define WF_EMPTY_BLOCK(count, per) do { if (uint64_t(blockIdx.x) * uint64_t(per) >= uint64_t(count)) return; } while (0)
-#define WF_DYN(a) do { if ((a).dyn) { (a).st = (a).dyn->st; (a).slotMap = (a).dyn->slotMap; } } while (0)
 
 __device__ __forceinline__ void wfPush(uint32_t* q, uint32_t* counter, bool pred, uint32_t slot) {
   const unsigned long long m = __ballot(pred);
@@ -144,6 +136,37 @@
     uint32_t d = dummies;
     for (int o = 32; o > 0; o >>= 1) d += __shfl_down(d, o);
     if (lane == 0 && d) atomicAdd(&counters[WC_DUMMY], d);
+  }
+};
+constexpr uint32_t kMigrateWaves = 16;
+struct WfMigrateLds { uint32_t cur[kMigrateWaves], end[kMigrateWaves]; };
+struct WfMigrate {
+  uint32_t* cur; uint32_t* end;
+  uint32_t* counter;
+  uint32_t* map;
+  uint32_t base, cap, size;
+  __device__ __forceinline__ WfMigrate(WfMigrateLds& l, const WfArgs& a, uint32_t count, uint32_t nWaves)
+      : cur(&l.cur[threadIdx.x >> 6]), end(&l.end[threadIdx.x >> 6]), counter(&a.counters[WC_REGION + a.migRegion]), map(a.slotMap),
+        base(a.migOff), cap(a.migCap), size(regionRange(count, nWaves)) {
+    if ((threadIdx.x & 63u) == 0) { *cur = 0; *end = 0; }
+  }
+  __device__ __forceinline__ uint32_t take(bool goesOn, uint32_t slot) {
+    if (cap == 0u) return slot;
+    const unsigned long long m = __ballot(goesOn);
+    if (m == 0) return slot;
+    const uint32_t lane = threadIdx.x & 63u, n = uint32_t(__popcll(m));
+    const int leader = __ffsll((long long) m) - 1;
+    RegionTake t{kRegionNone, 0u, 0u};
+    if (int(lane) == leader) {
+      RegionRange r{*(volatile uint32_t*) cur, *(volatile uint32_t*) end};
+      t = regionAsk(r, n, size, cap, [&](uint32_t add) {
+        return __hip_atomic_load(counter, __ATOMIC_RELAXED, __HIP_MEMORY_SCOPE_AGENT) < cap ? atomicAdd(counter, add) : kRegionNone;
+      });
+      *(volatile uint32_t*) cur = r.cur; *(volatile uint32_t*) end = r.end;
+    }
+    t.first = __shfl(t.first, leader); t.nFirst = __shfl(t.nFirst, leader); t.second = __shfl(t.second, leader);
+    if (!goesOn || t.first == kRegionNone) return slot;
+    return base + regionSlot(t, uint32_t(__popcll(m & ((1ull << lane) - 1ull))));
   }
 };
 constexpr uint32_t kRetryStageCap = 128;
@@ -206,14 +229,12 @@
 
 template <int MODE>
 __global__ void __launch_bounds__(kBlock, 6) k_wf_extend_fast(WfArgs a) {
-  WF_DYN(a);
   __shared__ uint64_t ldsStack[kWfLdsStackFast * kBlock];
   wfTraverseQueue<kWfLdsStackFast, false, true>(a, a.qA, a.counters[WC_ACTIVE], &a.counters[WC_CUR_EXTEND], ldsStack,
       [&](const TravStack& stk, uint32_t slot, WfTally& tally) { return !wfExtendFast<MODE>(a.sc, stk, a.st, slot, tally); });
 }
 template <bool RETRY>
 __global__ void __launch_bounds__(kBlock, 4) k_wf_extend(WfArgs a) {
-  WF_DYN(a);
   __shared__ uint64_t ldsStack[kWfLdsStack * kBlock];
   wfTraverseQueue<kWfLdsStack, true, false>(a, RETRY ? a.qR : a.qA, a.counters[RETRY ? WC_RETRY : WC_ACTIVE],
       &a.counters[RETRY ? WC_CUR_RETRY : WC_CUR_EXTEND], ldsStack,
@@ -221,7 +242,6 @@
 }
 template <int MODE>
 __global__ void __launch_bounds__(kBlock, 6) k_wf_shadow_fast(WfArgs a) {
-  WF_DYN(a);
   __shared__ uint64_t ldsStack[kWfLdsStackFast * kBlock];
   uint32_t rays = 0;
   wfTraverseQueue<kWfLdsStackFast, false, false>(a, a.qS, a.counters[WC_SHADOW], &a.counters[WC_CUR_SHADOW], ldsStack,
@@ -230,7 +250,6 @@
 }
 template <bool RETRY>
 __global__ void __launch_bounds__(kBlock, 4) k_wf_shadow(WfArgs a) {
-  WF_DYN(a);
   __shared__ uint64_t ldsStack[kWfLdsStack * kBlock];
   uint32_t rays = 0;
   __shared__ WfRepairLds repairLds;
@@ -247,7 +266,6 @@
 template <int MODE, int NODES>
 __global__ void __launch_bounds__(kBlock, leanWaves(MODE)) k_wf_extend_lean(WfArgs a) {
   WF_EMPTY_BLOCK(a.counters[WC_ACTIVE], kBlock);
-  WF_DYN(a);
   __shared__ uint64_t ldsStack[kWfLdsStackFast * kBlock];
   __shared__ uint32_t stageRetry[kBlock / 64][kRetryStageCap];
   const uint32_t gtid = blockIdx.x * blockDim.x + threadIdx.x;
@@ -281,7 +299,6 @@
 template <int MODE, int NODES>
 __global__ void __launch_bounds__(kBlock, leanWaves(MODE)) k_wf_shadow_lean(WfArgs a) {
   WF_EMPTY_BLOCK(a.counters[WC_SHADOW], kBlock);
-  WF_DYN(a);
   __shared__ uint64_t ldsStack[kWfLdsStackFast * kBlock];
   __shared__ uint32_t stageRetry[kBlock / 64][kRetryStageCap];
   const uint32_t gtid = blockIdx.x * blockDim.x + threadIdx.x;
@@ -322,7 +339,6 @@
 template <int NODES>
 __global__ void __launch_bounds__(kBlock, YART_RETRY_WAVES) k_wf_extend_retry_lean(WfArgs a) {
   WF_EMPTY_BLOCK(a.counters[WC_RETRY], kBlock);
-  WF_DYN(a);
   __shared__ uint64_t ldsStack[kWfLdsStack * kBlock];
   const uint32_t gtid = blockIdx.x * blockDim.x + threadIdx.x;
   TravStack stk;
@@ -361,7 +377,6 @@
 template <int NODES>
 __global__ void __launch_bounds__(kBlock, YART_RETRY_WAVES) k_wf_shadow_retry_lean(WfArgs a) {
   WF_EMPTY_BLOCK(a.counters[WC_RETRY], kBlock);
-  WF_DYN(a);
   __shared__ uint64_t ldsStack[kWfLdsStack * kBlock];
   const uint32_t gtid = blockIdx.x * blockDim.x + threadIdx.x;
   TravStack stk;
@@ -408,13 +423,13 @@
 #define YART_SHADE_WAVES 3
 #endif
 constexpr int kShadeBlock = YART_SHADE_WAVES * 256;
+static_assert(kShadeBlock / 64 <= int(kMigrateWaves), "WfMigrateLds: one row per wave");
 constexpr uint32_t kShadeStageCap = 512;
 constexpr int kShadeBlocksPerCU = 1;
 constexpr uint32_t kShadeHashSlots = 264, kShadeMatSlots = 64, kShadeTexSlots = 128, kShadeLightSlots = 8, kShadeEnvSlots = 4, kShadeNodeSlots = 32;
 template <bool SORT, bool FIT, bool ENV1>
 __global__ void __launch_bounds__(kShadeBlock, kShadeBlocksPerCU) k_wf_shade(WfArgs a) {
   WF_EMPTY_BLOCK(a.counters[0], kShadeBlock * 4);
-  WF_DYN(a);
   if (ENV1) { __builtin_assume(a.sc.nArea == 0u); __builtin_assume(a.sc.nInfinite == 1u); __builtin_assume(a.sc.nLights == 1u); }
   const uint32_t lane = threadIdx.x & 63u;
   const unsigned long long laneLt = (1ull << lane) - 1ull;
@@ -428,6 +443,11 @@
   uint32_t* mySorted = sorted[threadIdx.x >> 6];
   const uint32_t waveId = (blockIdx.x * blockDim.x + threadIdx.x) >> 6, nWaves = (gridDim.x * blockDim.x) >> 6;
   uint32_t nSorted = 0;
+  __shared__ WfMigrateLds migLds;
+  WfMigrate mig(migLds, a, count, nWaves);
+#if defined(YART_COUNT_TRAVERSAL)
+  uint32_t nMoved = 0, nStayed = 0;
+#endif
   __shared__ uint64_t sHash[kShadeHashSlots];
   __shared__ uint32_t sSobol1[8 * 256];
   if (FIT || (a.rc.sampler.tab.hash != nullptr && a.rc.sampler.tab.dims + 3u <= kShadeHashSlots)) {
@@ -515,22 +535,25 @@
     uint32_t slot = 0;
     const bool valid = SORT ? (sub * 64u + lane < nSorted) : (k < count && a.qA[k] != kWfFreeSlot);
     if (valid) {
-      slot = SORT ? mySorted[sub * 64u + lane] : a.qA[k];
+      const uint32_t from = SORT ? mySorted[sub * 64u + lane] : a.qA[k];
       WfPath p;
-      WfShadeResult r = wfShade(a.sc, a.rc, sobol, a.st, slot, p, rays, tally);
+      WfNext nx;
+      WfShadeResult r = wfShade(a.sc, a.rc, sobol, a.st, from, p, rays, tally, a.poolSlots != 0u, mig, nx);
+      slot = nx.w;
+      toNext = nx.toNext;
+      if (nx.moved) a.slotMap[slot] = nx.mapWord;
       if (r == WF_SHADOW) {
         toShadow = true;
-        if (p.flags & WF_FINAL) toNext = false;
-        else if ((p.flags & WF_DEPTH_MASK) <= 1u) toNext = true;
-        else toNext = !a.poolSlots && wfRouletteTentative(a.rc, p);
         wfStoreThr(a.st, slot, p);
-      } else if (r == WF_CONTINUE && wfRoulette(a.rc, p)) {
+      } else if (r == WF_CONTINUE) {
         wfStoreThr(a.st, slot, p);
-        toNext = true;
       } else if (r != WF_SKIPPED) {
         const uint32_t segs = (p.flags & WF_DEPTH_MASK) + (r == WF_TERMINATED ? 1u : 0u);
         wfRetire(a.L, a.slotMap, p.slot, mk4(p.L.x, p.L.y, p.L.z, asF(segs + ((p.flags & WF_NEE_MASK) >> WF_NEE_SHIFT))), a.poolSlots != 0u);
       }
+#if defined(YART_COUNT_TRAVERSAL)
+      if (nx.moved) nMoved++; else if (toNext && a.migCap != 0u) nStayed++;
+#endif
     }
     if (!a.poolSlots) sNext.push(a.qB, &a.counters[1], toNext, slot);
     sShadow.push(a.qS, &a.counters[2], toShadow, slot);
@@ -545,5 +568,7 @@
   wfFlushTally(a.stats, tally);
 #if defined(YART_COUNT_TRAVERSAL)
   wfAddStat(a.stats + 28, rays);
-#endif
-}
+  wfAddStat(a.stats + 12, nMoved);
+  wfAddStat(a.stats + 13, nStayed);
+#endif
+}
diff --git a/yart_amd/csrc/yart_hip.hip b/yart_amd/csrc/yart_hip.hip
--- a/yart_amd/csrc/yart_hip.hip
+++ b/yart_amd/csrc/yart_hip.hip
@@ -265,9 +265,7 @@
   std::vector<unsigned long long> tileRaysHost;
   DevBuf<uint64_t> spill; DevBuf<float> hdr; DevBuf<uint32_t> probeIn; DevBuf<float> probeOut;
   DevBuf<f4> wf[9];
-  DevBuf<f4> wfTail[1][9];
-  DevBuf<uint32_t> wfTailMap[2];
-  DevBuf<WfDyn> wfDyn;
+  DevBuf<uint32_t> wfMap;
   DevBuf<unsigned long long> pathsLog;
   DevBuf<f4> aovAcc[3], aovRec; DevBuf<uint32_t> aovRays; DevBuf<int32_t> aovIds; DevBuf<uint32_t> aovOut;
   DevBuf<MomentState> momState; DevBuf<uint32_t> momOut;
@@ -479,6 +477,7 @@
   size_t aovStride;
   size_t slots;
   uint32_t poolSlots, resumeCap;
+  uint32_t regions, regionCapDiv;
 };
 
 struct BatchBudget { uint64_t maxPaths, poolFit; };
@@ -493,12 +492,11 @@
     if (const char* e = std::getenv("YART_FAKE_FREE_MB")) freeB = size_t(std::max<long long>(1, std::atoll(e))) << 20;
     uint64_t held = uint64_t(s.L.n) * 16 + (uint64_t(s.qA.n) + s.qB.n + s.qS.n + s.qR.n) * 4 + uint64_t(s.resumeRec.n) * 16;
     for (auto& b : s.wf) held += uint64_t(b.n) * 16;
-    for (auto& t : s.wfTail) for (auto& b : t) held += uint64_t(b.n) * 16;
-    held += (uint64_t(s.wfTailMap[0].n) + s.wfTailMap[1].n) * 4;
+    held += uint64_t(s.wfMap.n) * 4;
     held += uint64_t(s.smpEntries.n) * 8;
     held += uint64_t(s.aovRec.n) * 16;
     if (std::getenv("YART_FAKE_FREE_MB")) held = 0;
-    const uint64_t perPath = (pl.compact ? 251 : 176) + ((p.flags & YART_FLAG_NO_RESUME) ? 0 : (kResumeWords * 16 + 7) / 8);
+    const uint64_t perPath = (pl.compact ? 32 + regionBytesPerPath(pl.regions) : 176) + ((p.flags & YART_FLAG_NO_RESUME) ? 0 : (kResumeWords * 16 + 7) / 8);
     const uint64_t dimsEst = std::min<uint32_t>(256u, (4u + 8u * p.max_depth + 16u + 7u) & ~7u);
     const uint64_t fixedB = uint64_t(nPix) * dimsEst * 8 + uint64_t(pl.gridMax) * kBlock * (kResumeWords * 16 + uint64_t(spillDepthFor(s.host, true)) * 8) +
                             (pl.mom ? uint64_t(nPix) * sizeof(MomentState) : 0u);
@@ -571,6 +569,12 @@
   pl.waveCap = std::max(std::min(p.first_wave_samples, p.samples), maxWave);
   pl.pool = !pl.mega && (p.flags & YART_FLAG_PATH_POOL) != 0;
   pl.compact = !pl.mega && !pl.pool && !(p.flags & YART_FLAG_NO_COMPACTION);
+  pl.regions = pl.compact ? YART_REGIONS : 0u;
+  pl.regionCapDiv = 1u;
+  if (pl.compact) {
+    if (const char* e = std::getenv("YART_REGION_COUNT")) pl.regions = uint32_t(std::min<long long>(kMaxRegions, std::max<long long>(1, std::atoll(e))));
+    if (const char* e = std::getenv("YART_REGION_CAP_DIV")) pl.regionCapDiv = uint32_t(std::min<long long>(1 << 20, std::max<long long>(1, std::atoll(e))));
+  }
   const BatchBudget fit = batchBudget(s, pl);
   pl.chunk = uint32_t(std::min<uint64_t>(pl.nPix ? pl.nPix : 1, std::max<uint64_t>(fit.maxPaths / pl.waveCap, 1)));
   if (pl.nPix > pl.chunk) {
@@ -615,13 +619,14 @@
     s.poolMap.ensure(pl.slots);
     if (!s.poolHost) HIP_CHECK(hipHostMalloc(reinterpret_cast<void**>(&s.poolHost), kPoolLag * WC_COUNT * sizeof(uint32_t)));
   }
-  for (auto& b : s.wf) b.ensure(pl.slots);
+  size_t arena = pl.slots;
   if (pl.compact) {
-    for (auto& b : s.wfTail[0]) b.ensure(pl.slots / 2 + 64);
-    s.wfTailMap[0].ensure(pl.slots / 2 + 64);
-    s.wfTailMap[1].ensure(pl.slots / 4 + 64);
-    s.wfDyn.ensure(1);
-  }
+    const RegionPlan rp = makeRegionPlan(uint32_t(pl.slots), pl.regions, pl.regionCapDiv);
+    if (!regionPlanFits(rp)) throw HipError("path-state arena: a queue word cannot index it (2^31 slots and more)");
+    arena = size_t(rp.end);
+    s.wfMap.ensure(arena);
+  }
+  for (auto& b : s.wf) b.ensure(arena);
   s.qA.ensure(pl.slots); s.qB.ensure(pl.slots); s.qS.ensure(pl.slots); s.qR.ensure(pl.slots); s.wfCounters.ensure(WC_COUNT);
   if (pl.resumeCap) s.resumeRec.ensure(size_t(pl.resumeCap) * kResumeWords);
 }
@@ -783,17 +788,10 @@
   AovArgs av = aovArgs(s, pl, b);
   WfArgs a = wfArgs(s, pl, b);
   const uint32_t maxDepth = pl.rc.maxDepth;
+  RegionPlan rp{};
   if (pl.compact) {
-    for (int k = 0; k < 2; k++) {
-      f4** f = &a.tail[k].ray0;
-      for (int j = 0; j < 9; j++) f[j] = k == 0 ? s.wfTail[0][j].p : s.wf[j].p;
-      a.tailMap[k] = s.wfTailMap[k].p;
-      a.tailCap[k] = a.nPaths / (k == 0 ? 2u : 4u);
-    }
-    WfDyn d0{};
-    d0.st = a.st; d0.slotMap = nullptr; d0.extent = a.nPaths; d0.inTail = 0;
-    HIP_CHECK(hipMemcpyAsync(s.wfDyn.p, &d0, sizeof(d0), hipMemcpyHostToDevice, stream));
-    a.dyn = s.wfDyn.p;
+    rp = makeRegionPlan(a.nPaths, pl.regions, pl.regionCapDiv);
+    a.slotMap = s.wfMap.p;
   }
   const uint32_t init[WC_COUNT] = {a.nPaths, 0, 0, 0, 0, 0, 0, 0, 0};
   HIP_CHECK(hipMemcpyAsync(s.wfCounters.p, init, sizeof(init), hipMemcpyHostToDevice, stream));
@@ -818,6 +816,9 @@
       }
       aovReduce(av, stream);
     }
+    const bool thinning = bounce >= 1 && bounce + 1 < maxDepth;
+    a.migCap = 0;
+    if (pl.compact && thinning && bounce - 1u < rp.k) { a.migRegion = bounce - 1u; a.migOff = rp.off[a.migRegion]; a.migCap = rp.cap[a.migRegion]; }
     {
       TraceRange rgShade("yart:shade", stream);
       shadeStage(pl, a, t, stream);
@@ -826,19 +827,11 @@
       TraceRange rgShadow("yart:shadow", stream);
       shadowStage(pl, a, t, stream);
     }
-    const bool thinning = bounce >= 1 && bounce + 1 < maxDepth;
     if (thinning) { TraceRange rgR("yart:roulette"); }
     hipLaunchKernelGGL(k_wf_advance, dim3(1), dim3(64), 0, stream, s.wfCounters.p, bounce + 1 < 16u ? s.pathsLog.p + bounce + 1 : nullptr);
     HIP_CHECK(hipGetLastError());
     std::swap(a.qA, a.qB);
-    if (pl.compact && thinning) {
-      TraceRange rgC("yart:compact", stream);
-      t.shade.begin(stream);
-      hipLaunchKernelGGL(k_wf_compact, dim3(s.numCUs * YART_STREAM_BLOCKS), dim3(kBlock), 0, stream, a);
-      hipLaunchKernelGGL(k_wf_compact_commit, dim3(1), dim3(64), 0, stream, a);
-      HIP_CHECK(hipGetLastError());
-      t.shade.end(stream);
-    }
+    if (pl.compact && thinning) { TraceRange rgC("yart:compact"); }
   }
 }
 
```

New measurement: 682.3 Msamples/s (median of 6 runs). About the same (+0.9%).
